# SixLabors/ZlibStream

Hardware: AMD Instinct MI355X
Metric: deflate MB/s (input) at level 6, 64 MiB buffers (higher is better)
Workload: dtype u8; 1 GPU; english64: 1 x 67108864-byte pseudo-random-English (Zipf words of alice29.txt) buffer per GPU, level 6, zlib framing, inputs resident in HBM; level=6, buffer_bytes=67108864, buffers_per_gpu=1, compressed_bytes=27425826, parallelism=independent buffers, 1 GPU(s), no collective in the data path

## Files before the change

zlibstream_amd/csrc/zs_engine.hip:

```cpp
#include <hip/hip_runtime.h>

#include <algorithm>
#include <cstdio>
#include <cstdlib>
#include <cstring>
#include <string>
#include <thread>
#include <vector>

#define ZS_BUILDING_LIBRARY
#include "../../include/zsgpu.h"
#include "zs_kernels.hip"
#include "zs_inflate_par.hip"
#include "zs_inflate_tok.hip"
#include "zs_png.hip"
#include "zs_crc32.hip"

using namespace zs;

namespace {

struct DevBuf {
    void *p = nullptr;
    size_t cap = 0;
};

enum Stage {
    kStClear, kStAdler, kStLinks, kStMatch, kStChunkMap, kStSegMap, kStResolve, kStExpand, kStEmitSyms, kStTail, kStTrees,
    kStOffsets, kStEmitBits, kStSpecWalk, kStSpecVerify, kStCrc32, kStSpecCompact, kStPngExpand, kStPngSplit, kStPngPack, kStPngSurvey, kStPngCompose, kStPngDiff, kStPngCrop, kStCount
};
const char *const kStageNames[kStCount] = {"clear", "adler", "links", "match", "chunkmap", "segmap", "resolve", "expand",
                                           "emit_syms", "tail", "trees", "offsets", "emit_bits", "spec_walk", "spec_verify", "crc32_frame",
                                           "spec_compact", "png_expand", "png_split", "png_pack", "png_survey", "png_compose", "png_diff", "png_crop"};

}

struct zs_ctx {
    int device = 0;
    hipStream_t stream = nullptr;
    hipStream_t aux = nullptr;
    hipEvent_t ev_fork = nullptr, ev_join = nullptr, ev_pre0 = nullptr, ev_pre = nullptr;
    hipEvent_t ev_spec[4] = {};
    std::string err;
    bool profiling = false;
    int fast_fallbacks = 0;
    int round_runs = 0;
    int cut_rounds = 0;
    int lit_fallbacks = 0;
    int spec_streams = 0, spec_fallbacks = 0, spec_wrong_chunks = 0;
    int spec_periodic = 0;
    int64_t dbg_blk_off = 0, dbg_chunk_off = 0, dbg_nchunks = 0, dbg_spec_n = 0, dbg_n_spec = 0;
    int64_t lit_engine_bytes = 0;
    std::vector<int64_t> inf_used;
    int64_t *inf_probe = nullptr;
    int inf_lane_streams = 0;
    int inf_wave_streams = 0;
    int64_t png_segments = 0;
    int fast_rounds = 0;
    bool no_rounds_once = false;
    int last_op = 0;
    hipEvent_t ev[kStCount + 1] = {};
    double stage_ms[kStCount] = {};
    uint32_t *crc_tab = nullptr;
    DevBuf sd, st, work, wpre, geo, link, mm, maps, chunk_far, segmap, supmap, seg_entry, seg_symbase, seg_stale, entry, symbase, stale, syms, blk_end, blk_top, blocks, trees, info, tile_bits, pieces, scratch,
        stage_in, stage_out, wr, inf_desc, inf_state, par_ps, par_st, par_work, par_cbits, par_ccnt, par_surv, par_scnt, par_cands, par_tabs, par_toktabs, par_toks, par_ctoks, par_tokstat, par_tails, par_retry, par_fxtab, par_blocks, par_cells,
        par_windows, par_fail, run_syms, run_bits, run_scratch, run_outs, run_fail, adl_tr, adl_res, plan_blk, ins_bits, mm_bak, cut_pos, cut_bkt, win_groups, win_sg, win_maps, win_entries, persist_bak, resume_flag, rle_tiles, own_in, fr_chunks, fr_meta, fr_planes, fr_prov, fr_base, fr_counters, spec_rec, spec_flags, spec_syms, png_img, png_seg, png_ctr, png_fimg, png_scratch, png_a7img, png_inflated, png_passes, crc_desc, crc_res, png_zs, png_gather, png_ximg, png_raw, png_simg, png_split, png_gimg, png_vimg, png_vrec, png_packed, png_cimg, png_frames, png_dimg, png_drec, png_kimg, png_crop;
    uint32_t *crc32_tab = nullptr;
    hipEvent_t ev_crc[2] = {};
    hipEvent_t ev_expand[2] = {};
    hipEvent_t ev_split[2] = {};
    hipEvent_t ev_pack[2] = {};
    hipEvent_t ev_survey[2] = {};
    hipEvent_t ev_compose[2] = {};
    hipEvent_t ev_diff[2] = {};
    hipEvent_t ev_crop[2] = {};
    bool resume_poisoned = false;
    void *pinned = nullptr;
    size_t pinned_cap = 0;
    void *pin_io = nullptr;
    size_t pin_io_cap = 0;
    bool pin_io_busy = false;
    void *pin_out = nullptr;
    size_t pin_out_cap = 0;
    bool pin_out_busy = false;
};

namespace {

bool fail(zs_ctx *c, const char *what, hipError_t e) {
    c->err = std::string(what) + ": " + hipGetErrorString(e);
    return false;
}
#define ZS_HIP(c, call)                                  \
    do {                                                 \
        hipError_t e_ = (call);                          \
        if (e_ != hipSuccess) return fail(c, #call, e_); \
    } while (0)

bool ensure(zs_ctx *c, DevBuf &b, size_t bytes) {
    if (bytes <= b.cap) return true;
    if (b.p) (void)hipFree(b.p);
    b.p = nullptr;
    b.cap = 0;
    size_t want = bytes + bytes / 8 + 4096;
    if (hipMalloc(&b.p, want) != hipSuccess) {
        (void)hipGetLastError();
        b.p = nullptr;
        want = bytes + 4096;
        if (hipMalloc(&b.p, want) != hipSuccess) {
            (void)hipGetLastError();
            b.p = nullptr;
            char msg[160];
            snprintf(msg, sizeof msg, "workspace: %zu bytes do not fit the device's free memory (the pipeline needs ~17 bytes per input byte: split the batch)", bytes);
            c->err = msg;
            return false;
        }
    }
    b.cap = want;
    return true;
}
bool ensure_pinned(zs_ctx *c, size_t bytes) {
    if (bytes <= c->pinned_cap) return true;
    if (c->pinned) (void)hipHostFree(c->pinned);
    c->pinned = nullptr;
    c->pinned_cap = 0;
    ZS_HIP(c, hipHostMalloc(&c->pinned, bytes + 4096, hipHostMallocDefault));
    c->pinned_cap = bytes + 4096;
    return true;
}

struct WorkList {
    std::vector<int32_t> pre;
    void add(int stream, int64_t count) {
        while ((int)pre.size() <= stream) pre.push_back(pre.empty() ? 0 : pre.back());
        pre.push_back(pre.back() + (int32_t)count);
    }
    void finish(int n) {
        if (pre.empty()) pre.push_back(0);
        while ((int)pre.size() <= n) pre.push_back(pre.back());
    }
    size_t size() const { return pre.empty() ? 0 : (size_t)pre.back(); }
    bool empty() const { return size() == 0; }
};
constexpr int kWorkLists = 9;
struct Plan {
    std::vector<StreamDesc> sd;
    WorkList w_clear, w_adler, w_links, w_match, w_chunks, w_segs, w_sups, w_blocks, w_runs;
    int64_t n_pos = 0, n_syms = 0;
    int64_t n_chunks = 0, n_segs = 0, n_sups = 0, n_blocks = 0, n_pieces = 0, n_runs = 0;
    int64_t n_spec = 0;
    int max_spec_n = 0, n_spec_streams = 0;
    bool any_fv = false, any_rle = false;
    bool any_dual = false;
    int64_t n_rle_tiles = 0;
    int64_t lit_bytes = 0;
    std::vector<FsChunk> fr_chunks;
    size_t fr_prov = 0;
    int fr_max_n = 0;
    int64_t n_cuts = 0;
    std::vector<int32_t> seg_c0, seg_after, seg_base, seg_S, seg_cl, cstart, head;
    std::vector<uint32_t> cl;
    std::vector<BlockRec> plan_blk;
    std::vector<int32_t> plan_wr_blk;
};

template <class T>
T *dev(DevBuf &b) {
    return (T *)b.p;
}

struct WriteSpec {
    std::vector<int64_t> ends;
    std::vector<uint8_t> flush;
    int chunk = 512;
    bool raw = false;
    bool flushing() const {
        for (uint8_t f : flush)
            if (f) return true;
        return false;
    }
};

struct RunOpts {
    bool final_run = true, cont = false;
    int64_t hist = 0;
    LitPersist *persist = nullptr;
    int64_t abs_off = 0;
    uint32_t adler_stream = 1, carry_byte = 0;
    int64_t end_bits = 0;
    int64_t stop_abs = -1;
    bool resume = false, mid_write = false, at_read = false;
    int64_t p0 = 0, E0 = 0, base0 = 0, start_block = 0;
    int slot = 0;
    uint32_t start_syms = 0;
};

bool run_pipeline(zs_ctx *c, int n, const void *const *in, const int64_t *in_len, void *const *out, const int64_t *out_cap,
                  int64_t *out_len, int *status, int level, int strategy, int hash_variant, hipStream_t stream,
                  const WriteSpec *const *writes = nullptr, int force_seq = 0, RunOpts *ro = nullptr, bool rounds = false,
                  const std::vector<uint8_t> *force_lit = nullptr) {
    if (level == -1) level = 6;
    LevelCfg lv = level_cfg(level);
    static const bool host_times = getenv("ZS_HOST_TIMES") != nullptr;
    const auto ht0 = std::chrono::steady_clock::now();
    auto ht_us = [&]() { return std::chrono::duration<double, std::micro>(std::chrono::steady_clock::now() - ht0).count(); };
    double ht_plan = 0, ht_launched = 0;
    for (int i = 0; i < n; i++) {
        out_len[i] = 0;
        if (status) status[i] = ZS_STREAM_ERROR;
    }
    bool any_writes = false;
    for (int i = 0; i < n && writes; i++) any_writes = any_writes || writes[i] != nullptr;
    if (any_writes && n > 1)
        for (int i = 0; i < n; i++)
            if (ro || (writes[i] && writes[i]->flushing())) {
                c->err = "flush modes and incremental runs take one stream a call";
                return false;
            }
    std::vector<WriteSpec> rle_one;
    std::vector<const WriteSpec *> rle_writes;
    if (any_writes && strategy == kRle && level >= 1 && !ro && !getenv("ZS_NO_RLE_MULTI")) {
        rle_one.resize((size_t)n);
        rle_writes.assign(writes, writes + n);
        for (int i = 0; i < n; i++) {
            const WriteSpec *wr = writes[i];
            if (!wr || wr->ends.size() <= 1 || wr->flushing()) continue;
            bool safe = true;
            for (size_t k = 0; k + 1 < wr->ends.size() && safe; k++) {
                const int64_t E = wr->ends[k];
                safe = !(E >= kWindowSize - kMinLookahead && (E % kWSize) >= kWSize - kMinLookahead);
            }
            if (safe) {
                rle_one[(size_t)i] = *wr;
                rle_one[(size_t)i].ends.assign(1, in_len[i]);
                rle_one[(size_t)i].flush.assign(1, 0);
                rle_writes[(size_t)i] = &rle_one[(size_t)i];
            }
        }
        writes = rle_writes.data();
    }
    static const int64_t fast_min_input = getenv("ZS_FAST_MIN_INPUT") ? atoll(getenv("ZS_FAST_MIN_INPUT")) : kFastMinPeriodic;
    bool allow_dual = lv.func == 1 && strategy != kRle && strategy != kHuffmanOnly && !any_writes && !ro && !rounds && force_seq == 0 && !force_lit && n <= 16 && !getenv("ZS_NO_FAST_VEC") &&
                      !getenv("ZS_FAST_NO_ROUNDS");
    for (int i = 0; i < n && allow_dual; i++) allow_dual = in_len[i] >= fast_min_input && in_len[i] < kFastMinInput;
    bool dual_broken = false;
    const bool spec_on = !getenv("ZS_NO_SPEC");
    const int spec_len_env = getenv("ZS_SPEC_LEN") ? atoi(getenv("ZS_SPEC_LEN")) : 0;
    const int spec_bits = spec_len_env == 512 ? 9 : spec_len_env == 2048 ? 11 : spec_len_env == 1024 ? 10 : kSpecLenBits;
    const int spec_warm = getenv("ZS_SPEC_WARM") ? std::max(0, std::min(4096, atoi(getenv("ZS_SPEC_WARM")))) : kSpecWarm;
    const int64_t spec_min = getenv("ZS_SPEC_MIN") ? std::max<int64_t>(kWindowSize, atoll(getenv("ZS_SPEC_MIN"))) : kSpecMinInput;
    const int spec_corrupt = getenv("ZS_SPEC_CORRUPT") ? atoi(getenv("ZS_SPEC_CORRUPT")) : -1;
plan_again:
    Plan pl;
    pl.sd.resize((size_t)n);
    int64_t total_len = 0;
    for (int i = 0; i < n; i++) total_len += in_len[i];
    const int64_t link_span = total_len >= (48ll << 20) ? 262144 : total_len >= (24ll << 20) ? 131072 : 65536;
    const int run_chunk = getenv("ZS_FAST_CHUNK") ? std::max(65536, std::min((int)kFastChunk, atoi(getenv("ZS_FAST_CHUNK")) & ~65535))
                                                  : (int)std::max<int64_t>(65536, std::min<int64_t>(kFastChunk, ((total_len / 256 + 65535) >> 16) << 16));
    for (int i = 0; i < n; i++) {
        StreamDesc &s = pl.sd[(size_t)i];
        int64_t len = in_len[i];
        const WriteSpec *const wr = writes ? writes[i] : nullptr;
        s.in = (const uint8_t *)in[i];
        s.out = (uint8_t *)out[i];
        s.out_cap = out_cap[i];
        s.n = (int32_t)len;
        const bool multi = wr && wr->ends.size() > 1;
        const bool flushing = wr && (wr->flushing() || ro);
        const bool resume = ro && ro->resume;
        const bool cont = ro && ro->cont && !resume, final_run = !ro || ro->final_run;
        std::vector<ReadEvent> rev;
        Geometry geo;
        const int64_t one_write[1] = {len};
        const bool real_flush = wr && wr->flushing();
        const bool lit_forced = force_lit && (*force_lit)[(size_t)i];
        const std::vector<int64_t> no_ends_;
        GeoStart gs;
        if (resume) gs.resume = true, gs.at_read = ro->at_read, gs.p0 = ro->p0, gs.E0 = ro->E0, gs.base0 = ro->base0;
        bool inner_flush = false;
        if (wr)
            for (size_t k = 0; k + 1 < wr->flush.size(); k++) inner_flush = inner_flush || wr->flush[k] != 0;
        const bool slow_ok = lv.func == 2 && strategy != kRle && !cont && !lit_forced && !(multi && inner_flush) &&
                             build_geometry(len, multi ? wr->ends : no_ends_, geo, gs);
        const bool fast_multi = multi && !inner_flush && !cont && !resume && lv.func == 1 && strategy != kRle && !getenv("ZS_NO_FAST_MULTI") &&
                                build_read_events(len, wr->ends, rev, true);
        const bool fast_resume = resume && ro->at_read && lv.func == 1 && strategy != kRle && !inner_flush && !lit_forced && !getenv("ZS_NO_FAST_RESUME") &&
                                 len - ro->p0 >= 2 * kMinLookahead &&
                                 (multi ? build_read_events(len, wr->ends, rev, true, ro->p0, ro->base0)
                                        : build_read_events(len, std::vector<int64_t>(one_write, one_write + 1), rev, true, ro->p0, ro->base0));
        const bool regular = fast_resume ? true : cont ? false : multi ? fast_multi : build_read_events(len, std::vector<int64_t>(one_write, one_write + 1), rev);
        s.body_end = slow_ok ? (int32_t)geo.body_end : -1;
        const bool fast_one = lv.func == 1 && strategy != kRle && regular && len >= kMinLookahead && !cont && !resume &&
                              ((!flushing && final_run && !ro && (!multi || fast_multi)) || (ro && (!multi || fast_multi) && !inner_flush && !lit_forced && !getenv("ZS_NO_FAST_RESUME")));
        const bool fast_par = fast_one && !multi && force_seq != 1 && !ro && strategy != kHuffmanOnly &&
                              (len >= kFastMinInput || allow_dual || (force_seq == 2 && n <= 16 && len >= fast_min_input));
        if (allow_dual && !fast_par) dual_broken = true;
        s.fv_end = ((fast_one && (!fast_par || allow_dual) && !getenv("ZS_NO_FAST_VEC")) || fast_resume) ? (int32_t)(len - kMinLookahead) : -1;
        s.ins_bits = nullptr;
        if (s.fv_end >= 0) {
            pl.any_fv = true;
        }
        s.rle_end = -1, s.rle_tile_off = 0;
        s.fr_first = 0, s.fr_n = 0;
        if (strategy == kRle && level >= 1 && !multi && !flushing && final_run && !ro && regular && !getenv("ZS_NO_RLE_RUNS")) {
            s.rle_end = (int32_t)rle_body_end(len);
            if (s.rle_end >= 0) {
                pl.any_rle = true;
                s.rle_tile_off = (int32_t)pl.n_rle_tiles;
                pl.n_rle_tiles += (s.rle_end + kMaxMatch + 1 + 4095) / 4096;
            }
        }
        s.n_wr = (multi || flushing) ? (int32_t)wr->ends.size() : 1;
        s.wr_end = nullptr;
        s.wr_flush = nullptr, s.wr_blk = nullptr, s.out_chunk = wr ? wr->chunk : 512, s.raw = wr && wr->raw;
        s.kl = num_refills(len - (resume ? ro->base0 : 0));
        s.resume = resume && (slow_ok || fast_resume) ? 1 : 0, s.cont_bits = (cont || resume) ? 1 : 0, s.mid_write = (ro && (ro->mid_write || (resume && !ro->at_read))) ? 1 : 0;
        if (resume && !slow_ok && !fast_resume) {
            c->err = "the run cannot go on in the bulk pipeline from where the literal engine stopped";
            return false;
        }
        s.start_slot = resume ? ro->slot : 0, s.start_syms = resume ? ro->start_syms : 0, s.base0 = resume ? ro->base0 : 0;
        s.start_block = resume ? ro->start_block : 0, s.start_pos = resume ? ro->p0 : 0, s.persist_off = resume ? ro->abs_off : 0, s.stop_abs = (ro && cont) ? ro->stop_abs : -1;
        s.nchunks = s.body_end >= 0 ? geo.nchunks() : 0;
        s.pos_off = pl.n_pos;
        pl.n_pos += (len + 64 + 63) & ~63LL;
        s.sym_off = pl.n_syms;
        pl.n_syms += len + 64 + (ro ? kLitBufsize : 0);
        s.chunk_off = (int32_t)pl.n_chunks;
        pl.n_chunks += s.nchunks;
        s.seg_off = (int32_t)pl.n_segs;
        s.nsegs = 0;
        s.cut_off = (int32_t)pl.n_cuts, s.cut_cap = 0;
        s.grid_chunks = 0;
        if (s.body_end >= 0) {
            s.grid_chunks = 1;
            for (size_t k = 1; k + 1 < geo.cstart.size() && s.grid_chunks; k++)
                if (geo.cstart[k] != (int32_t)((int64_t)k * kChunk - (kMinLookahead - 1))) s.grid_chunks = 0;
            if (geo.cstart.empty() || geo.cstart[0] != 0) s.grid_chunks = 0;
            for (size_t k = 0; k < geo.head.size() && s.grid_chunks; k++)
                if (geo.head[k] != ((k >= 32 && ((k - 32) & 15) == 0) ? (int32_t)((k - 32) >> 4) + 2 : 0)) s.grid_chunks = 0;
            s.cut_cap = (int32_t)(geo.cl.size() + (size_t)geo.nsegs() + 8);
            pl.n_cuts += s.cut_cap;
            s.nsegs = geo.nsegs();
            const int32_t cl0 = (int32_t)pl.cl.size();
            pl.seg_c0.insert(pl.seg_c0.end(), geo.seg_c0.begin(), geo.seg_c0.end());
            pl.seg_after.insert(pl.seg_after.end(), geo.seg_after.begin(), geo.seg_after.end());
            pl.seg_base.insert(pl.seg_base.end(), geo.seg_base.begin(), geo.seg_base.end());
            pl.seg_S.insert(pl.seg_S.end(), geo.seg_S.begin(), geo.seg_S.end());
            for (int32_t v : geo.seg_cl) pl.seg_cl.push_back(v + cl0);
            pl.cl.insert(pl.cl.end(), geo.cl.begin(), geo.cl.end());
            pl.cstart.insert(pl.cstart.end(), geo.cstart.begin(), geo.cstart.end());
            pl.head.insert(pl.head.end(), geo.head.begin(), geo.head.end());
        } else {
            if (fast_resume) {
                pl.seg_c0.push_back(0), pl.seg_after.push_back((int32_t)std::max<int64_t>(ro->p0, kMinLookahead - 1)), pl.seg_base.push_back((int32_t)ro->base0);
                pl.seg_S.push_back(0), pl.seg_cl.push_back((int32_t)pl.cl.size());
                s.nsegs++;
            }
            if (s.fv_end >= 0 || s.rle_end >= 0)
                for (size_t k = 0; k < rev.size(); k++) {
                    const int64_t at = (k || fast_resume) ? rev[k].at - (s.rle_end >= 0 ? kMaxMatch : kMinLookahead - 1) : 0;
                    if (at > (s.rle_end >= 0 ? s.rle_end : s.fv_end)) break;
                    pl.seg_c0.push_back(0), pl.seg_after.push_back((int32_t)rev[k].after), pl.seg_base.push_back((int32_t)rev[k].base);
                    pl.seg_S.push_back(0), pl.seg_cl.push_back((int32_t)pl.cl.size());
                    s.nsegs++;
                }
            pl.seg_cl.push_back((int32_t)pl.cl.size());
            pl.cstart.push_back(0);
        }
        s.seg_c0 = s.seg_after = s.seg_base = s.seg_S = s.seg_cl = nullptr, s.cl = nullptr, s.cstart = nullptr, s.head = nullptr;
        pl.n_segs += s.nsegs;
        s.sup_off = (int32_t)pl.n_sups;
        pl.n_sups += (s.nsegs + kSupSegs - 1) / kSupSegs;
        s.spec = 0, s.spec_n = 0, s.spec_off = (int32_t)pl.n_spec;
        bool spec_geo = s.body_end >= 0 && geo.body_end == len - kMinLookahead;
        if (spec_geo) {
            const int64_t want = 1 + (len > kWindowSize ? (len - kWindowSize - 1) / kWSize + 1 : 0);
            spec_geo = (int64_t)geo.nsegs() == want && geo.seg_cl.size() == (size_t)want + 1 && geo.seg_cl[0] == 0 && geo.seg_cl[1] == 0;
            for (int64_t k = 1; k < want && spec_geo; k++)
                spec_geo = geo.seg_cl[(size_t)k + 1] - geo.seg_cl[(size_t)k] == 1 &&
                           geo.cl[(size_t)geo.seg_cl[(size_t)k]] == ((uint32_t)(kWindowSize + kWSize * (k - 1)) | kClWindowBit);
        }
        if (spec_on && lv.func == 2 && (strategy == kDefault || strategy == kFiltered) && !wr && !ro && !lit_forced && spec_geo && len >= spec_min &&
            n <= 65535) {
            s.spec = 1, s.spec_n = (int32_t)((((int64_t)s.body_end + kMinLookahead - 1) >> spec_bits) + 1);
            pl.n_spec += s.spec_n, pl.n_spec_streams++;
            pl.max_spec_n = std::max(pl.max_spec_n, (int)s.spec_n);
        }
        s.run_chunk = run_chunk;
        s.fast_runs = fast_par ? (force_seq == 2 ? 1 : (int32_t)((len + run_chunk - 1) / run_chunk)) : 0;
        s.run_slots = fast_par ? (force_seq == 2 ? (int32_t)((len + 4096) / kFastChunk + 1) : s.fast_runs) : 0;
        s.run_off = (int32_t)pl.n_runs;
        pl.n_runs += s.run_slots;
        pl.w_runs.add(i, s.fast_runs);
        s.blk_off = (int32_t)pl.n_blocks;
        s.max_blocks = (int32_t)(level == 0 ? len / 8191 + len / 32506 + 4 : len / kBlockSyms + 2);
        if (flushing) s.max_blocks += (int32_t)wr->ends.size() + 1;
        s.plan_blk = nullptr, s.plan_nblk = 0;
        s.final_run = final_run ? 1 : 0, s.cont = cont ? 1 : 0, s.persist = ro ? ro->persist : nullptr;
        s.abs_off = (ro && !resume) ? ro->abs_off : 0, s.adler_stream = ro ? ro->adler_stream : 1, s.carry_byte = ro ? ro->carry_byte : 0;
        if (level == 0 && strategy != kRle && !ro) {
            const size_t first = pl.plan_blk.size();
            const std::vector<int64_t> no_ends;
            const std::vector<uint8_t> no_flush;
            if (flushing) pl.plan_wr_blk.assign(wr->ends.size(), 0);
            plan_stored_blocks(len, (multi || flushing) ? wr->ends : no_ends, flushing ? wr->flush : no_flush,
                               [&](int64_t start, int32_t blen, int can_store, int eof) {
                                   pl.plan_blk.push_back(BlockRec{start, 0, blen, 0, can_store, eof});
                               },
                               [&](int w, int nb) {
                                   if (flushing) pl.plan_wr_blk[(size_t)w] = nb;
                               });
            s.plan_nblk = (int32_t)(pl.plan_blk.size() - first);
            s.plan_blk = (const BlockRec *)(uintptr_t)first;
            s.max_blocks = s.plan_nblk + 1;
        }
        pl.n_blocks += s.max_blocks;
        s.adler_off = (int32_t)pl.n_pieces;
        s.n_adler = ro ? 0 : (int32_t)((len + kAdlerPiece - 1) / kAdlerPiece);
        pl.n_pieces += s.n_adler;
        pl.w_clear.add(i, (s.out_cap + 65535) / 65536);
        pl.w_adler.add(i, s.n_adler);
        if (s.body_end >= 0 || s.fast_runs > 0 || s.fv_end >= 0)
            pl.w_links.add(i, len - 5 > 0 ? (len - 5 + link_span - 1) / link_span : 0);
        if (s.body_end >= 0) {
            pl.w_match.add(i, (int64_t)s.body_end / kMatchTile + 1);
            pl.w_chunks.add(i, s.nchunks);
            pl.w_segs.add(i, s.nsegs);
            if (s.nsegs > kSupSegs) pl.w_sups.add(i, (s.nsegs + kSupSegs - 1) / kSupSegs);
        }
        pl.w_blocks.add(i, s.max_blocks);
        if (s.body_end < 0 && s.fv_end < 0 && s.rle_end < 0 && s.fast_runs == 0 && s.plan_nblk == 0 && !(level == 0 && strategy != kRle && !ro)) {
            const int64_t from = resume ? ro->p0 : ro ? ro->hist : 0;
            pl.lit_bytes += std::max<int64_t>(0, len - from - (kMinLookahead - 1));
        }
    }
    {
        int64_t need = 0;
        for (int i = 0; i < n; i++) need += (pl.sd[(size_t)i].spec_n + 63) / 64;
        if (pl.n_spec && (int64_t)((pl.max_spec_n + 63) / 64) * n > 4 * need + 4096) {
            for (int i = 0; i < n; i++) pl.sd[(size_t)i].spec = 0, pl.sd[(size_t)i].spec_n = 0, pl.sd[(size_t)i].spec_off = 0;
            pl.n_spec = 0, pl.max_spec_n = 0, pl.n_spec_streams = 0;
        }
    }
    if (allow_dual && dual_broken) {
        allow_dual = false, dual_broken = false;
        goto plan_again;
    }
    pl.any_dual = allow_dual;
    c->lit_engine_bytes += pl.lit_bytes;
    auto plan_rerun = [&]() { c->lit_engine_bytes -= pl.lit_bytes; };
    c->fast_rounds = 0;
    const bool no_rounds_this_call = c->no_rounds_once;
    c->no_rounds_once = false;
    if (pl.any_fv && !getenv("ZS_FAST_NO_ROUNDS") && !no_rounds_this_call && !(ro && ro->resume && getenv("ZS_NO_RESUME_ROUNDS"))) {
        int64_t pos_fv = 0, max_fv = 0;
        for (int i = 0; i < n; i++)
            if (pl.sd[(size_t)i].fv_end >= 0) {
                pos_fv += pl.sd[(size_t)i].fv_end + 1 - pl.sd[(size_t)i].start_pos;
                max_fv = std::max<int64_t>(max_fv, pl.sd[(size_t)i].fv_end + 1 - pl.sd[(size_t)i].start_pos);
            }
        const double t_stream = (double)max_fv / (level >= 3 ? 20e6 : level == 2 ? 35e6 : 46e6);
        const double t_rounds = std::min(0.016, (double)max_fv / 60e6) + (double)pos_fv / 3.5e9;
        if (getenv("ZS_FR_RATIO") ? (double)pos_fv <= atof(getenv("ZS_FR_RATIO")) * (double)max_fv : t_rounds < t_stream) {
            int64_t target = getenv("ZS_FR_CHUNK") ? atoll(getenv("ZS_FR_CHUNK")) : pos_fv / 250;
            target = target < 2048 ? 2048 : target > kFsChunkMax ? kFsChunkMax : target;
            bool too_short = false;
            for (;;) {
                pl.fr_chunks.clear();
                pl.fr_max_n = 0;
                too_short = false;
                for (int i = 0; i < n; i++) {
                    StreamDesc &s = pl.sd[(size_t)i];
                    if (s.fv_end < 0) continue;
                    s.fr_first = (int32_t)pl.fr_chunks.size();
                    {
                        const int32_t *after = pl.seg_after.data() + s.seg_off;
                        const bool res = s.resume != 0;
                        const int64_t shortest = fs_build_chunks(i, (int64_t)s.fv_end, s.nsegs - 1, [&](int k) { return (int64_t)after[k - 1] - (kMinLookahead - 1); }, (int)target, pl.fr_chunks,
                                                                 res ? 2 : 1, res ? s.start_pos : 0);
                        if (shortest < kFsMinSpan) too_short = true;
                    }
                    s.fr_n = (int32_t)pl.fr_chunks.size() - s.fr_first;
                    pl.fr_max_n = s.fr_n > pl.fr_max_n ? s.fr_n : pl.fr_max_n;
                }
                if (pl.fr_chunks.size() <= 256 || target >= kFsChunkMax || getenv("ZS_FR_CHUNK")) break;
                target += 128;
            }
            if (too_short) {
                pl.fr_chunks.clear();
                pl.fr_max_n = 0;
                for (int i = 0; i < n; i++) pl.sd[(size_t)i].fr_first = pl.sd[(size_t)i].fr_n = 0;
            }
            for (FsChunk &ck : pl.fr_chunks) {
                ck.prov_off = (uint32_t)pl.fr_prov;
                pl.fr_prov += (size_t)(ck.b_hi - ck.b_lo) + kMaxMatch + 64;
            }
            if (pl.fr_prov > 0xFFFF0000u) {
                pl.fr_chunks.clear();
                pl.fr_max_n = 0, pl.fr_prov = 0;
                for (int i = 0; i < n; i++) pl.sd[(size_t)i].fr_first = pl.sd[(size_t)i].fr_n = 0;
            }
        }
    }
    WorkList *const lists[kWorkLists] = {&pl.w_clear, &pl.w_adler, &pl.w_links, &pl.w_match, &pl.w_chunks, &pl.w_segs, &pl.w_sups, &pl.w_blocks, &pl.w_runs};
    for (WorkList *l : lists) l->finish(n);
    size_t n_work = pl.w_clear.size() + pl.w_adler.size() + pl.w_links.size() + pl.w_match.size() + pl.w_chunks.size() +
                    pl.w_segs.size() + pl.w_sups.size() + pl.w_blocks.size() + pl.w_runs.size();
    if (!ensure(c, c->sd, sizeof(StreamDesc) * (size_t)n) || !ensure(c, c->st, sizeof(StreamState) * (size_t)n) ||
        !ensure(c, c->work, sizeof(uint2) * (n_work + 1)) || !ensure(c, c->link, 2 * (size_t)pl.n_pos + 64) ||
        !ensure(c, c->mm, 8 * (size_t)pl.n_pos + 256) ||
        !ensure(c, c->maps, 4 * (size_t)(pl.n_chunks + 1) * kSlots) || !ensure(c, c->segmap, 8 * (size_t)(pl.n_segs + 1) * kSlots) ||
        !ensure(c, c->supmap, 8 * (size_t)(pl.n_sups + 1) * kSlots) || !ensure(c, c->chunk_far, 2 * (size_t)pl.n_chunks + 64) ||
        !ensure(c, c->seg_entry, 2 * (size_t)(pl.n_segs + 2)) || !ensure(c, c->seg_symbase, 4 * (size_t)(pl.n_segs + 2)) ||
        !ensure(c, c->seg_stale, (size_t)pl.n_segs + 64) || !ensure(c, c->entry, 2 * (size_t)(pl.n_chunks + 2)) ||
        !ensure(c, c->symbase, 4 * (size_t)(pl.n_chunks + 2)) || !ensure(c, c->stale, (size_t)pl.n_chunks + 64) ||
        !ensure(c, c->syms, 4 * (size_t)pl.n_syms + kSymsSlack) || !ensure(c, c->blk_end, 4 * (size_t)pl.n_blocks + 64) ||
        !ensure(c, c->blk_top, 4 * (size_t)pl.n_blocks + 64) || !ensure(c, c->blocks, sizeof(BlockRec) * (size_t)pl.n_blocks) ||
        !ensure(c, c->trees, sizeof(TreeWork) * (size_t)pl.n_blocks) || !ensure(c, c->info, sizeof(BlockInfo) * (size_t)pl.n_blocks) ||
        !ensure(c, c->tile_bits, 4 * (size_t)kEbTiles * (size_t)pl.n_blocks + 64) ||
        !ensure(c, c->pieces, 4 * (size_t)pl.n_pieces + 64) || !ensure(c, c->scratch, (size_t)kScratchBytes * (size_t)n) ||
        !ensure(c, c->cut_pos, 8 * (size_t)pl.n_cuts + 64) || !ensure(c, c->cut_bkt, 8 * (size_t)pl.n_cuts + 64) ||
        (pl.n_spec && (!ensure(c, c->spec_rec, 8 * (size_t)pl.n_spec + 64) || !ensure(c, c->spec_flags, 4 * (size_t)n + 64) ||
                       !ensure(c, c->spec_syms, 4 * (size_t)pl.n_spec * (size_t)spec_slab_stride(spec_bits) + 64))))
        return false;
    const size_t o_segcl = 16 * (size_t)pl.n_segs, o_cstart = o_segcl + 4 * ((size_t)pl.n_segs + (size_t)n),
                 o_head = o_cstart + 4 * ((size_t)pl.n_chunks + (size_t)n), o_cl = o_head + 4 * (size_t)pl.n_chunks;
    const size_t geo_bytes = o_cl + 4 * pl.cl.size();
    if (!ensure(c, c->geo, geo_bytes + 64)) return false;
    for (int i = 0; i < n; i++) {
        StreamDesc &s = pl.sd[(size_t)i];
        const int32_t *g = (const int32_t *)c->geo.p;
        const uint8_t *gb = (const uint8_t *)c->geo.p;
        s.seg_c0 = g + s.seg_off, s.seg_after = g + pl.n_segs + s.seg_off, s.seg_base = g + 2 * pl.n_segs + s.seg_off;
        s.seg_S = g + 3 * pl.n_segs + s.seg_off;
        s.seg_cl = (const int32_t *)(gb + o_segcl) + s.seg_off + i;
        s.cstart = (const int32_t *)(gb + o_cstart) + s.chunk_off + i;
        s.head = (const int32_t *)(gb + o_head) + s.chunk_off;
        s.cl = (const uint32_t *)(gb + o_cl);
    }
    if (pl.any_fv) {
        if (!ensure(c, c->ins_bits, (size_t)pl.n_pos / 8 + kFvBitSlack)) return false;
        for (int i = 0; i < n; i++)
            if (pl.sd[(size_t)i].fv_end >= 0) pl.sd[(size_t)i].ins_bits = dev<uint32_t>(c->ins_bits) + pl.sd[(size_t)i].pos_off / 32;
    }
    if (!pl.plan_blk.empty()) {
        if (!ensure(c, c->plan_blk, sizeof(BlockRec) * pl.plan_blk.size())) return false;
        for (int i = 0; i < n; i++)
            if (pl.sd[(size_t)i].plan_nblk) pl.sd[(size_t)i].plan_blk = dev<BlockRec>(c->plan_blk) + (uintptr_t)pl.sd[(size_t)i].plan_blk;
    }
    if (pl.n_runs &&
        (!ensure(c, c->run_syms, 4 * (size_t)pl.n_runs * kFastRunSyms) || !ensure(c, c->run_bits, 4 * (size_t)pl.n_runs * kFastRunBitWords) ||
         !ensure(c, c->run_scratch, (size_t)pl.n_runs * kFastRunScratch) || !ensure(c, c->run_outs, sizeof(FastRunOut) * (size_t)pl.n_runs) ||
         !ensure(c, c->run_fail, 4 * (size_t)n + 64)))
        return false;
    if (any_writes) {
        std::vector<size_t> nws((size_t)n, 0), offs;
        for (int i = 0; i < n; i++) {
            const WriteSpec *wr = writes[i];
            if (wr && (wr->ends.size() > 1 || wr->flushing() || ro)) nws[(size_t)i] = wr->ends.size();
        }
        const size_t wr_bytes = layout_write_blocks(nws, offs);
        if (!ensure(c, c->wr, wr_bytes + 64)) return false;
        std::vector<uint8_t> hw(rounds ? 0 : wr_bytes + 64, 0);
        for (int i = 0; i < n; i++) {
            const WriteSpec *wr = writes[i];
            const size_t nw = nws[(size_t)i];
            if (!wr || !(wr->ends.size() > 1 || wr->flushing() || ro)) continue;
            uint8_t *blk = (uint8_t *)c->wr.p + offs[(size_t)i];
            pl.sd[(size_t)i].wr_end = (const int64_t *)blk;
            if (wr->flushing() || ro) {
                pl.sd[(size_t)i].wr_blk = (int32_t *)(blk + 8 * nw);
                pl.sd[(size_t)i].wr_flush = blk + 12 * nw;
            }
            if (rounds || !nw) continue;
            memcpy(hw.data() + offs[(size_t)i], wr->ends.data(), sizeof(int64_t) * nw);
            if (wr->flushing() || ro) memcpy(hw.data() + offs[(size_t)i] + 12 * nw, wr->flush.data(), nw);
            if (!pl.plan_wr_blk.empty()) memcpy(hw.data() + offs[(size_t)i] + 8 * nw, pl.plan_wr_blk.data(), 4 * nw);
        }
        if (!rounds && wr_bytes) {
            ZS_HIP(c, hipMemcpyAsync(c->wr.p, hw.data(), hw.size(), hipMemcpyHostToDevice, stream));
            ZS_HIP(c, hipStreamSynchronize(stream));
        }
    }
    if (!rounds && !pl.plan_blk.empty()) {
        ZS_HIP(c, hipMemcpyAsync(c->plan_blk.p, pl.plan_blk.data(), sizeof(BlockRec) * pl.plan_blk.size(), hipMemcpyHostToDevice, stream));
        ZS_HIP(c, hipStreamSynchronize(stream));
    }
    const size_t pre_bytes = 4 * (size_t)kWorkLists * (size_t)(n + 1);
    size_t up_bytes = sizeof(StreamDesc) * (size_t)n + pre_bytes + geo_bytes + 16;
    if (!ensure_pinned(c, std::max(up_bytes, sizeof(StreamState) * (size_t)n)) || !ensure(c, c->wpre, pre_bytes + 64)) return false;
    uint8_t *hp = (uint8_t *)c->pinned;
    memcpy(hp, pl.sd.data(), sizeof(StreamDesc) * (size_t)n);
    int32_t *hpre = (int32_t *)(hp + sizeof(StreamDesc) * (size_t)n);
    size_t o_clear = 0, o_adler, o_links, o_match, o_chunks, o_segs, o_sups, o_blocks, o_runs;
    WorkOffsets wo;
    {
        size_t *const offs[kWorkLists] = {&o_clear, &o_adler, &o_links, &o_match, &o_chunks, &o_segs, &o_sups, &o_blocks, &o_runs};
        size_t at = 0;
        for (int l = 0; l < kWorkLists; l++) {
            *offs[l] = at;
            wo.off[l] = (uint32_t)at;
            memcpy(hpre + (size_t)l * (size_t)(n + 1), lists[l]->pre.data(), 4 * (size_t)(n + 1));
            at += lists[l]->size();
        }
        wo.off[kWorkLists] = (uint32_t)at;
    }
    if (geo_bytes) {
        uint8_t *hg = hp + sizeof(StreamDesc) * (size_t)n + pre_bytes;
        if (pl.n_segs) {
            memcpy(hg, pl.seg_c0.data(), 4 * (size_t)pl.n_segs);
            memcpy(hg + 4 * (size_t)pl.n_segs, pl.seg_after.data(), 4 * (size_t)pl.n_segs);
            memcpy(hg + 8 * (size_t)pl.n_segs, pl.seg_base.data(), 4 * (size_t)pl.n_segs);
            memcpy(hg + 12 * (size_t)pl.n_segs, pl.seg_S.data(), 4 * (size_t)pl.n_segs);
        }
        memcpy(hg + o_segcl, pl.seg_cl.data(), 4 * pl.seg_cl.size());
        memcpy(hg + o_cstart, pl.cstart.data(), 4 * pl.cstart.size());
        if (pl.n_chunks) memcpy(hg + o_head, pl.head.data(), 4 * (size_t)pl.n_chunks);
        if (!pl.cl.empty()) memcpy(hg + o_cl, pl.cl.data(), 4 * pl.cl.size());
        if (!rounds) ZS_HIP(c, hipMemcpyAsync(c->geo.p, hg, geo_bytes, hipMemcpyHostToDevice, stream));
    }
    if (!rounds) ZS_HIP(c, hipMemcpyAsync(c->sd.p, hp, sizeof(StreamDesc) * (size_t)n, hipMemcpyHostToDevice, stream));
    if (n_work && !rounds) {
        ZS_HIP(c, hipMemcpyAsync(c->wpre.p, hpre, pre_bytes, hipMemcpyHostToDevice, stream));
        hipLaunchKernelGGL(zs_worklist_kernel, dim3((unsigned)((n_work + 255) / 256)), dim3(256), 0, stream, dev<int32_t>(c->wpre), n, wo,
                           dev<uint2>(c->work));
    }
    if (!rounds) {
        ZeroRegions z;
        auto reg = [&](int r, DevBuf &b, size_t bytes) {
            z.p[r] = b.p;
            z.n16[r] = (uint32_t)(((bytes + 15) / 16 < b.cap / 16) ? (bytes + 15) / 16 : b.cap / 16);
        };
        reg(0, c->stale, (size_t)pl.n_chunks + 64);
        reg(1, c->seg_stale, (size_t)pl.n_segs + 64);
        reg(2, c->st, sizeof(StreamState) * (size_t)n);
        if (pl.any_fv) reg(3, c->ins_bits, (size_t)pl.n_pos / 8 + kFvBitSlack);
        else z.p[3] = nullptr, z.n16[3] = 0;
        uint32_t most = 0;
        for (int r = 0; r < 4; r++) most = z.n16[r] > most ? z.n16[r] : most;
        unsigned blocks = (most + 255) / 256;
        if (blocks > 2048) blocks = 2048;
        if (blocks < 1) blocks = 1;
        hipLaunchKernelGGL(zs_zero_kernel, dim3(blocks), dim3(256), 0, stream, z);
        if (ro && ro->resume && pl.sd[0].fv_end >= 0) {
            const int64_t lo = std::max<int64_t>(0, ro->p0 - kWSize - 64) / 32, hi = ro->p0 / 32;
            if (hi > lo) ZS_HIP(c, hipMemsetAsync(pl.sd[0].ins_bits + lo, 0xFF, (size_t)(hi - lo) * 4, stream));
            ZS_HIP(c, hipMemsetD32Async((hipDeviceptr_t)(pl.sd[0].ins_bits + hi), (int)((1u << (ro->p0 & 31)) - 1u), 1, stream));
        }
    }

    const StreamDesc *d_sd = dev<StreamDesc>(c->sd);
    StreamState *d_st = dev<StreamState>(c->st);
    const uint2 *d_work = dev<uint2>(c->work);
    const bool prof = c->profiling;
    const int k5_ahead = getenv("ZS_K5_AHEAD") ? atoi(getenv("ZS_K5_AHEAD")) : 1;
    c->dbg_blk_off = pl.sd[0].blk_off, c->dbg_chunk_off = pl.sd[0].chunk_off, c->dbg_nchunks = pl.sd[0].nchunks;
    c->dbg_spec_n = pl.sd[0].spec_n, c->dbg_n_spec = pl.n_spec;
    const K5Spec k5s{dev<uint32_t>(c->spec_rec), dev<uint32_t>(c->spec_rec) + pl.n_spec, spec_bits, spec_warm, spec_corrupt,
                     dev<uint32_t>(c->spec_syms), spec_slab_stride(spec_bits)};
    int spec_ok_streams = 0;
    bool need_maps = true, spec_ran = false;
    if (!rounds) c->spec_streams = c->spec_fallbacks = c->spec_wrong_chunks = c->spec_periodic = 0;
    auto mark = [&](int i) {
        if (prof) (void)hipEventRecord(c->ev[i], stream);
    };
    ht_plan = ht_us();
    ZS_HIP(c, hipEventRecord(c->ev_pre0, stream));
    auto side_work = [&]() -> bool {
        ZS_HIP(c, hipStreamWaitEvent(c->aux, c->ev_pre0, 0));
        if (!pl.w_clear.empty())
            hipLaunchKernelGGL(zs_clear_kernel, dim3((unsigned)pl.w_clear.size()), dim3(256), 0, c->aux, d_sd, d_work + o_clear);
        if (!pl.w_adler.empty())
            hipLaunchKernelGGL(zs_adler_kernel, dim3((unsigned)pl.w_adler.size()), dim3(256), 0, c->aux, d_sd, d_work + o_adler,
                               dev<uint32_t>(c->pieces));
        ZS_HIP(c, hipEventRecord(c->ev_pre, c->aux));
        return true;
    };
    const int cut_budget = getenv("ZS_FORCE_ROUNDS") ? 0 : kCutBudget;
    const int defer_mode = ((ro || getenv("ZS_NO_DEFER")) ? 0 : 1) | (getenv("ZS_DEBUG_CUTS") ? 0x100 : 0) | (cut_budget << 16);
    const int cut_stride = (int)pl.n_cuts;
    const bool use_sup = !pl.w_sups.empty() && !getenv("ZS_NO_SUPMAP");
    auto launch_resolve = [&](int mode, int iter) {
        hipLaunchKernelGGL(zs_resolve_kernel, dim3((unsigned)n), dim3(1024), kResolveLds, stream, d_sd, d_st, dev<uint16_t>(c->link),
                           dev<uint2>(c->mm), dev<uint32_t>(c->maps), dev<uint2>(c->segmap),
                           dev<uint16_t>(c->seg_entry), dev<uint32_t>(c->seg_symbase), dev<uint8_t>(c->stale),
                           dev<uint8_t>(c->seg_stale), c->crc_tab, lv, strategy, hash_variant, 0x7FFFFFFF, 0x7FFFFFFF,
                           use_sup ? dev<uint2>(c->supmap) : (const uint2 *)nullptr, dev<uint16_t>(c->chunk_far), mode, dev<int32_t>(c->cut_pos),
                           dev<uint32_t>(c->cut_bkt), cut_stride, iter);
    };
    auto run_cut_rounds = [&]() -> bool {
        const size_t far_off = 8 * (size_t)pl.n_pos + 256;
        if (!ensure(c, c->mm_bak, far_off + 2 * (size_t)pl.n_chunks + 64)) return false;
        ZS_HIP(c, hipMemcpyAsync(c->mm_bak.p, c->mm.p, 8 * (size_t)pl.n_pos + 256, hipMemcpyDeviceToDevice, stream));
        ZS_HIP(c, hipMemcpyAsync((uint8_t *)c->mm_bak.p + far_off, c->chunk_far.p, 2 * (size_t)pl.n_chunks + 64, hipMemcpyDeviceToDevice, stream));
        ZS_HIP(c, hipMemsetAsync(c->cut_pos.p, 0xFF, 8 * (size_t)pl.n_cuts + 64, stream));
        StreamState *hr = (StreamState *)c->pinned;
        for (int iter = 0;; iter++) {
            launch_resolve(3 | (defer_mode & 0x100), iter);
            ZS_HIP(c, hipMemcpyAsync(hr, d_st, sizeof(StreamState) * (size_t)n, hipMemcpyDeviceToHost, stream));
            ZS_HIP(c, hipStreamSynchronize(stream));
            bool all_same = true;
            int max_nc = 0;
            for (int i = 0; i < n; i++)
                if (hr[i].deferred == 1 && !hr[i].cuts_same) all_same = false, max_nc = std::max(max_nc, hr[i].nc[iter & 1]);
            hipLaunchKernelGGL(zs_cuts_apply_kernel, dim3((unsigned)n), dim3(256), 0, stream, d_sd, d_st, dev<uint16_t>(c->link), dev<int32_t>(c->cut_pos),
                               cut_stride, iter);
            if (getenv("ZS_DEBUG")) {
                int nd = 0, nsame = 0;
                for (int i = 0; i < n; i++) nd += hr[i].deferred == 1, nsame += hr[i].deferred == 1 && hr[i].cuts_same;
                fprintf(stderr, "zs: cut round %d: %d streams in the rounds, %d settled, most cuts %d, stream 0: %d cuts, first difference at cut %d (position %d)\n", iter,
                        nd, nsame, max_nc, hr[0].nc[iter & 1], hr[0].cut_diff_idx, hr[0].cut_diff_pos);
            }
            if (all_same && getenv("ZS_DEBUG_CUTS")) {
                const int ncap = hr[0].nc[iter & 1];
                std::vector<int32_t> cp((size_t)ncap);
                std::vector<uint32_t> cb((size_t)ncap);
                (void)hipMemcpy(cp.data(), dev<int32_t>(c->cut_pos) + (size_t)(iter & 1) * (size_t)cut_stride + pl.sd[0].cut_off, 4 * (size_t)ncap, hipMemcpyDeviceToHost);
                (void)hipMemcpy(cb.data(), dev<uint32_t>(c->cut_bkt) + (size_t)(iter & 1) * (size_t)cut_stride + pl.sd[0].cut_off, 4 * (size_t)ncap, hipMemcpyDeviceToHost);
                fprintf(stderr, "zs: cuts of stream 0 (slot: position / bucket):");
                for (int k = 0; k < ncap; k++)
                    if (cp[(size_t)k] >= 0) fprintf(stderr, " %d: %d / %u", k, cp[(size_t)k], cb[(size_t)k]);
                fprintf(stderr, "\n");
            }
            if (all_same) break;
            if (iter >= 4096) {
                c->err = "the cut rounds did not settle";
                return false;
            }
            c->cut_rounds++;
            if (iter > 0)
            hipLaunchKernelGGL(zs_cut_restore_kernel, dim3(2048, (unsigned)std::min(n, 65535)), dim3(256), 0, stream, d_sd, d_st, dev<uint2>(c->mm), (const uint2 *)c->mm_bak.p,
                               dev<uint8_t>(c->stale), dev<uint8_t>(c->seg_stale), dev<uint16_t>(c->chunk_far), (const uint16_t *)((const uint8_t *)c->mm_bak.p + far_off), n);
            if (max_nc > 0) {
                if (max_nc <= 64)
                    hipLaunchKernelGGL((zs_cuts_repair_kernel<256, 1>), dim3(128, (unsigned)max_nc, (unsigned)std::min(n, 65535)), dim3(256), kRepairLds, stream, d_sd, d_st,
                                       dev<uint16_t>(c->link), dev<uint2>(c->mm), dev<uint8_t>(c->stale), dev<uint8_t>(c->seg_stale),
                                       dev<uint16_t>(c->chunk_far), c->crc_tab, lv, hash_variant, dev<int32_t>(c->cut_pos), dev<uint32_t>(c->cut_bkt),
                                       cut_stride, iter, n);
                else if (max_nc <= 2048)
                    hipLaunchKernelGGL((zs_cuts_repair_kernel<256, 8>), dim3(16, (unsigned)max_nc, (unsigned)std::min(n, 65535)), dim3(256), kRepairLds, stream, d_sd, d_st,
                                       dev<uint16_t>(c->link), dev<uint2>(c->mm), dev<uint8_t>(c->stale), dev<uint8_t>(c->seg_stale),
                                       dev<uint16_t>(c->chunk_far), c->crc_tab, lv, hash_variant, dev<int32_t>(c->cut_pos), dev<uint32_t>(c->cut_bkt),
                                       cut_stride, iter, n);
                else
                    hipLaunchKernelGGL((zs_cuts_repair_kernel<1024, 32>), dim3(1, (unsigned)std::min(max_nc, 65535), (unsigned)std::min(n, 65535)), dim3(1024), kRepairLds, stream, d_sd,
                                       d_st, dev<uint16_t>(c->link), dev<uint2>(c->mm), dev<uint8_t>(c->stale), dev<uint8_t>(c->seg_stale),
                                       dev<uint16_t>(c->chunk_far), c->crc_tab, lv, hash_variant, dev<int32_t>(c->cut_pos), dev<uint32_t>(c->cut_bkt),
                                       cut_stride, iter, n);
            }
            hipLaunchKernelGGL(zs_chunkmap_kernel, dim3((unsigned)pl.w_chunks.size()), dim3(512), 0, stream, d_sd, d_work + o_chunks,
                               dev<uint2>(c->mm), dev<uint16_t>(c->link), dev<uint32_t>(c->maps), c->crc_tab, lv, strategy,
                               hash_variant, dev<uint16_t>(c->chunk_far), dev<uint8_t>(c->stale), (const StreamState *)d_st);
            hipLaunchKernelGGL(zs_segmap_kernel, dim3((unsigned)pl.w_segs.size()), dim3(320), 0, stream, d_sd, d_work + o_segs,
                               dev<uint32_t>(c->maps), dev<uint2>(c->segmap));
            ZS_HIP(c, hipMemsetAsync(c->seg_stale.p, 0, (size_t)pl.n_segs + 64, stream));
            if (use_sup)
                hipLaunchKernelGGL(zs_supmap_kernel, dim3((unsigned)pl.w_sups.size()), dim3(320), 0, stream, d_sd, d_work + o_sups,
                                   dev<uint2>(c->segmap), dev<uint8_t>(c->seg_stale), dev<uint2>(c->supmap));
        }
        return true;
    };
    if (!rounds) {
    mark(2);
    if (!pl.w_links.empty())
        hipLaunchKernelGGL(zs_links_kernel, dim3((unsigned)pl.w_links.size()), dim3(1024), kLkLds, stream, d_sd, d_work + o_links,
                           dev<uint16_t>(c->link), c->crc_tab, hash_variant, (int)link_span);
    if (ro && ro->resume)
        hipLaunchKernelGGL(zs_import_chains_kernel, dim3(64), dim3(1024), 0, stream, d_sd, 0, dev<uint16_t>(c->link), c->crc_tab, hash_variant, ro->p0);
    if (pl.any_dual) {
        bool periodic = true;
        if (!getenv("ZS_FAST_NO_PROBE")) {
            hipLaunchKernelGGL(zs_fast_probe_kernel, dim3((unsigned)n), dim3(256), 0, stream, d_sd, dev<uint16_t>(c->link), dev<int32_t>(c->run_fail));
            std::vector<int32_t> np((size_t)n, 0);
            ZS_HIP(c, hipMemcpyAsync(np.data(), c->run_fail.p, 4 * (size_t)n, hipMemcpyDeviceToHost, stream));
            ZS_HIP(c, hipStreamSynchronize(stream));
            for (int i = 0; i < n; i++) periodic = periodic && np[(size_t)i] == 0;
        }
        for (int i = 0; i < n; i++) {
            StreamDesc &sk = pl.sd[(size_t)i];
            if (periodic) sk.fv_end = -1, sk.fr_first = 0, sk.fr_n = 0;
            else sk.fast_runs = 0, sk.run_slots = 0;
        }
        if (periodic) pl.any_fv = false, pl.fr_chunks.clear(), pl.fr_max_n = 0;
        else pl.n_runs = 0;
        memcpy(c->pinned, pl.sd.data(), sizeof(StreamDesc) * (size_t)n);
        ZS_HIP(c, hipMemcpyAsync(c->sd.p, c->pinned, sizeof(StreamDesc) * (size_t)n, hipMemcpyHostToDevice, stream));
        if (getenv("ZS_DEBUG")) fprintf(stderr, "zs: %d stream(s) below 4 MiB at level %d: %s\n", n, level, periodic ? "all period, the speculative runs" : "the sweeps");
    }
    mark(3);
    if (strategy == kHuffmanOnly) {
        ZS_HIP(c, hipMemsetAsync(c->mm.p, 0, 8 * (size_t)pl.n_pos + 64, stream));
    } else if (!pl.w_match.empty())
        hipLaunchKernelGGL(zs_match_kernel, dim3((unsigned)pl.w_match.size()), dim3(1024), kMatchLds + 16, stream, d_sd, d_work + o_match,
                           dev<uint16_t>(c->link), dev<uint2>(c->mm), lv, strategy, d_st);
    mark(4);
    if (!side_work()) return false;
    if (pl.n_spec) {
        spec_ran = true;
        hipLaunchKernelGGL((zs_emit_syms_lane_kernel<4, 1>), dim3((unsigned)((pl.max_spec_n + 63) / 64), (unsigned)n), dim3(kK5Threads), 0, stream, d_sd, d_st,
                           (const uint2 *)nullptr, 0, dev<uint2>(c->mm), dev<uint16_t>(c->link), (const uint16_t *)nullptr, (const uint32_t *)nullptr,
                           (uint32_t *)nullptr, (int32_t *)nullptr, (int32_t *)nullptr, c->crc_tab, lv, strategy, hash_variant, k5_ahead, k5s);
        if (prof) (void)hipEventRecord(c->ev_spec[0], stream);
        hipLaunchKernelGGL(zs_spec_verify_kernel, dim3((unsigned)n), dim3(1024), 0, stream, d_sd, d_st, dev<uint2>(c->mm), dev<uint16_t>(c->link), c->crc_tab, lv,
                           strategy, hash_variant, k5s, dev<int32_t>(c->spec_flags));
        int32_t *hf = (int32_t *)c->pinned;
        ZS_HIP(c, hipMemcpyAsync(hf, c->spec_flags.p, 4 * (size_t)n, hipMemcpyDeviceToHost, stream));
        ZS_HIP(c, hipStreamSynchronize(stream));
        if (prof) (void)hipEventRecord(c->ev_spec[1], stream);
        for (int i = 0; i < n; i++) {
            if (hf[i] == 0) continue;
            c->spec_streams++;
            if (hf[i] == 1) spec_ok_streams++;
            else c->spec_fallbacks++;
            if (hf[i] == 2) c->spec_periodic++;
        }
        if (spec_ok_streams < c->spec_streams) {
            StreamState *hs = (StreamState *)c->pinned;
            ZS_HIP(c, hipMemcpyAsync(hs, d_st, sizeof(StreamState) * (size_t)n, hipMemcpyDeviceToHost, stream));
            ZS_HIP(c, hipStreamSynchronize(stream));
            for (int i = 0; i < n; i++) c->spec_wrong_chunks += hs[i].spec_wrong;
        }
        if (getenv("ZS_DEBUG"))
            fprintf(stderr, "zs: speculative walk: %d streams tried, %d verified, %d wrong guesses (chunks of %d, warm-up %d)\n", c->spec_streams, spec_ok_streams,
                    c->spec_wrong_chunks, 1 << spec_bits, spec_warm);
    }
    need_maps = spec_ok_streams < n;
    const StreamState *spec_st = spec_ok_streams ? (const StreamState *)d_st : nullptr;
    if (!pl.w_chunks.empty() && need_maps)
        hipLaunchKernelGGL(zs_chunkmap_kernel, dim3((unsigned)pl.w_chunks.size()), dim3(512), 0, stream, d_sd, d_work + o_chunks,
                           dev<uint2>(c->mm), dev<uint16_t>(c->link), dev<uint32_t>(c->maps), c->crc_tab, lv, strategy,
                           hash_variant, dev<uint16_t>(c->chunk_far), (uint8_t *)nullptr, (const StreamState *)nullptr, spec_st);
    mark(5);
    if (!pl.w_segs.empty() && need_maps)
        hipLaunchKernelGGL(zs_segmap_kernel, dim3((unsigned)pl.w_segs.size()), dim3(320), 0, stream, d_sd, d_work + o_segs,
                           dev<uint32_t>(c->maps), dev<uint2>(c->segmap), spec_st);
    if (use_sup && need_maps)
        hipLaunchKernelGGL(zs_supmap_kernel, dim3((unsigned)pl.w_sups.size()), dim3(320), 0, stream, d_sd, d_work + o_sups,
                           dev<uint2>(c->segmap), dev<uint8_t>(c->seg_stale), dev<uint2>(c->supmap), spec_st);
    mark(6);
    if (need_maps) launch_resolve(defer_mode, 0);
    }
    mark(7);
    if (pl.any_fv) {
        constexpr int fs_lds = fs_lds_bytes<1024, kFsTile1>();
        if (!pl.fr_chunks.empty()) {
            const size_t nch = pl.fr_chunks.size(), plane_words = (size_t)pl.n_pos / 32 + kFvBitSlack / 4 + 64;
            static const int env_max_rounds = getenv("ZS_FR_MAX_ROUNDS") ? atoi(getenv("ZS_FR_MAX_ROUNDS")) : 0;
            static const int env_range = getenv("ZS_FR_RANGE") ? std::max(1, atoi(getenv("ZS_FR_RANGE"))) : 0;
            static const int env_group = getenv("ZS_FR_GROUP") ? atoi(getenv("ZS_FR_GROUP")) : 4;
            static const int env_tail = getenv("ZS_FR_TAIL_RANGE") ? atoi(getenv("ZS_FR_TAIL_RANGE")) : 1;
            static const bool env_no_seed = getenv("ZS_FR_NO_SEED") != nullptr, env_fixed = getenv("ZS_FR_RANGE_FIXED") != nullptr, env_dbg = getenv("ZS_DEBUG") != nullptr;
            const int max_rounds = env_max_rounds ? env_max_rounds : pl.fr_max_n + 2;
            if (!ensure(c, c->fr_chunks, nch * sizeof(FsChunk)) || !ensure(c, c->fr_meta, 2 * nch * sizeof(FsMeta)) || !ensure(c, c->fr_planes, 16 * plane_words) ||
                !ensure(c, c->fr_prov, 4 * pl.fr_prov + 64) || !ensure(c, c->fr_base, 4 * nch + 64) || !ensure(c, c->fr_counters, 4 * ((size_t)max_rounds + 16))) {
                c->err.clear();
                ZS_HIP(c, hipStreamSynchronize(c->aux));
                ZS_HIP(c, hipStreamSynchronize(stream));
                c->no_rounds_once = true;
                return plan_rerun(), run_pipeline(c, n, in, in_len, out, out_cap, out_len, status, level, strategy, hash_variant, stream, writes, force_seq, ro, false, force_lit);
            }
            ZS_HIP(c, hipMemcpyAsync(c->fr_chunks.p, pl.fr_chunks.data(), nch * sizeof(FsChunk), hipMemcpyHostToDevice, stream));
            ZS_HIP(c, hipMemsetAsync(c->fr_counters.p, 0, 4 * ((size_t)max_rounds + 16), stream));
            const int range_max = env_range ? env_range : nch >= 512 ? (int)((nch + 255) / 256) : 1;
            FsRounds fr{dev<FsChunk>(c->fr_chunks), dev<FsMeta>(c->fr_meta), dev<uint32_t>(c->fr_planes), dev<uint32_t>(c->fr_prov), dev<uint32_t>(c->fr_counters),
                        (int64_t)plane_words, (int)nch, 0, env_no_seed ? 1 : 0, range_max};
            const int group = env_group;
            uint32_t changed = 1;
            int r = 0;
            std::string trace;
            while (r < max_rounds && changed) {
                const int g_n = fr.range > 1 ? 1 : group;
                const unsigned n_wg = (unsigned)((nch + (size_t)fr.range - 1) / (size_t)fr.range);
                for (int g = 0; g < g_n && r < max_rounds; g++, r++) {
                    fr.round = r;
                    hipLaunchKernelGGL((zs_fast_sweep_kernel<1024, kFsTile1, true>), dim3(n_wg), dim3(1024), fs_lds, stream, d_sd, d_st, dev<uint16_t>(c->link),
                                       dev<uint32_t>(c->syms), dev<int32_t>(c->blk_end), dev<int32_t>(c->blk_top), lv, strategy, fr);
                }
                ZS_HIP(c, hipMemcpyAsync(&changed, dev<uint32_t>(c->fr_counters) + (r - 1), 4, hipMemcpyDeviceToHost, stream));
                ZS_HIP(c, hipStreamSynchronize(stream));
                if (env_dbg) {
                    static auto t_last = std::chrono::steady_clock::now();
                    const auto t_now = std::chrono::steady_clock::now();
                    char b[64];
                    snprintf(b, sizeof b, " %u/%d(%.2f)", changed, fr.range, r <= g_n ? 0.0 : std::chrono::duration<double, std::milli>(t_now - t_last).count());
                    t_last = t_now;
                    trace += b;
                }
                if (!env_fixed) {
                    static const double env_wake = getenv("ZS_FR_WAKE") ? atof(getenv("ZS_FR_WAKE")) : 4.0;
                    const size_t awake = std::min<size_t>(nch, (size_t)(env_wake * (double)changed));
                    const int tail = env_tail;
                    fr.range = std::min<int>(range_max, std::max<int>(tail, (int)((awake + 255) / 256)));
                }
            }
            c->fast_rounds = r;
            if (env_dbg) fprintf(stderr, "zs: DeflateFast over %zu chunks of %d streams, up to %d to a workgroup: %d rounds (changed/range:%s)\n", nch, n, range_max, r, trace.c_str());
            if (changed) {
                ZS_HIP(c, hipStreamSynchronize(c->aux));
                c->no_rounds_once = true;
                return plan_rerun(), run_pipeline(c, n, in, in_len, out, out_cap, out_len, status, level, strategy, hash_variant, stream, writes, force_seq, ro, false, force_lit);
            }
            const FsMeta *mf = dev<FsMeta>(c->fr_meta) + (size_t)((r - 1) & 1) * nch;
            hipLaunchKernelGGL(zs_fast_commit_scan_kernel, dim3((unsigned)n), dim3(1024), 0, stream, d_sd, d_st, mf, dev<int32_t>(c->fr_base));
            hipLaunchKernelGGL(zs_fast_commit_kernel, dim3((unsigned)nch), dim3(256), 0, stream, d_sd, fr, mf, dev<int32_t>(c->fr_base), dev<uint16_t>(c->link),
                               dev<uint32_t>(c->syms), dev<int32_t>(c->blk_end), dev<int32_t>(c->blk_top));
        } else {
            hipLaunchKernelGGL((zs_fast_sweep_kernel<1024, kFsTile1, false>), dim3((unsigned)n), dim3(1024), fs_lds, stream, d_sd, d_st, dev<uint16_t>(c->link),
                               dev<uint32_t>(c->syms), dev<int32_t>(c->blk_end), dev<int32_t>(c->blk_top), lv, strategy, FsRounds());
        }
    }
    if (pl.any_rle) {
        const size_t nt = (size_t)pl.n_rle_tiles;
        if (!ensure(c, c->rle_tiles, 4 * (4 * nt + (size_t)n) + 256)) return false;
        int32_t *rb = dev<int32_t>(c->rle_tiles);
        RleTiles rt{rb, rb + nt, rb + 2 * nt, rb + 3 * nt, rb + 4 * nt};
        int max_tiles = 0;
        for (int i = 0; i < n; i++)
            if (pl.sd[(size_t)i].rle_end >= 0) max_tiles = std::max(max_tiles, (pl.sd[(size_t)i].rle_end + kMaxMatch + 1 + 4095) / 4096);
        auto tiles = [&](auto &&launch) {
            for (int s0 = 0; s0 < n; s0 += 65535) launch(dim3((unsigned)((max_tiles + 3) / 4), (unsigned)std::min(n - s0, 65535)), s0);
        };
        tiles([&](dim3 tg, int s0) { hipLaunchKernelGGL(zs_rle_starts_kernel, tg, dim3(256), 0, stream, d_sd, rt, s0); });
        hipLaunchKernelGGL(zs_rle_scan_kernel, dim3((unsigned)n), dim3(1024), 0, stream, d_sd, rt);
        tiles([&](dim3 tg, int s0) {
            hipLaunchKernelGGL(zs_rle_pass_kernel<0>, tg, dim3(256), 0, stream, d_sd, rt, dev<uint32_t>(c->syms), dev<int32_t>(c->blk_end), dev<int32_t>(c->blk_top), s0);
        });
        hipLaunchKernelGGL(zs_rle_sums_kernel, dim3((unsigned)n), dim3(1024), 0, stream, d_sd, d_st, rt);
        tiles([&](dim3 tg, int s0) {
            hipLaunchKernelGGL(zs_rle_pass_kernel<1>, tg, dim3(256), 0, stream, d_sd, rt, dev<uint32_t>(c->syms), dev<int32_t>(c->blk_end), dev<int32_t>(c->blk_top), s0);
        });
    }
    const bool tail_late = ro && (!ro->final_run || ro->resume);
    const bool tail_serial = !tail_late && n >= 64 && (pl.n_pos / n >= (96 << 10) || getenv("ZS_TAIL_SERIAL")) && !getenv("ZS_TAIL_FORK");
    if (!tail_late && !tail_serial) {
        ZS_HIP(c, hipEventRecord(c->ev_fork, stream));
        ZS_HIP(c, hipStreamWaitEvent(c->aux, c->ev_fork, 0));
        hipLaunchKernelGGL(zs_tail_kernel, dim3((unsigned)n), dim3(1024), kTailLds, c->aux, d_sd, d_st, dev<uint16_t>(c->link),
                           dev<uint32_t>(c->syms), dev<int32_t>(c->blk_end), dev<int32_t>(c->blk_top), dev<BlockRec>(c->blocks),
                           dev<uint8_t>(c->scratch), c->crc_tab, lv, strategy, hash_variant, level);
        ZS_HIP(c, hipEventRecord(c->ev_join, c->aux));
    }
    if (!pl.w_segs.empty() && need_maps)
        hipLaunchKernelGGL(zs_expand_kernel, dim3((unsigned)((pl.w_segs.size() + 63) / 64)), dim3(64), 0, stream, d_sd, d_st,
                           d_work + o_segs, (int)pl.w_segs.size(), dev<uint2>(c->mm), dev<uint16_t>(c->link),
                           dev<uint32_t>(c->maps), dev<uint16_t>(c->seg_entry), dev<uint32_t>(c->seg_symbase),
                           dev<uint8_t>(c->stale), dev<uint16_t>(c->entry), dev<uint32_t>(c->symbase), c->crc_tab, lv, strategy,
                           hash_variant);
    mark(8);
    if (!pl.w_chunks.empty() && need_maps)
        hipLaunchKernelGGL((zs_emit_syms_lane_kernel<4, 0>), dim3((unsigned)((pl.w_chunks.size() + 63) / 64)), dim3(kK5Threads), 0, stream, d_sd, d_st,
                           d_work + o_chunks, (int)pl.w_chunks.size(), dev<uint2>(c->mm), dev<uint16_t>(c->link), dev<uint16_t>(c->entry),
                           dev<uint32_t>(c->symbase), dev<uint32_t>(c->syms), dev<int32_t>(c->blk_end), dev<int32_t>(c->blk_top),
                           c->crc_tab, lv, strategy, hash_variant, k5_ahead, k5s);
    if (spec_ok_streams) {
        if (prof) (void)hipEventRecord(c->ev_spec[2], stream);
        hipLaunchKernelGGL(zs_spec_compact_kernel, dim3((unsigned)((pl.max_spec_n + 3) / 4), (unsigned)n), dim3(256), 0, stream, d_sd, d_st, k5s,
                           dev<uint32_t>(c->syms), dev<int32_t>(c->blk_end), dev<int32_t>(c->blk_top));
        if (prof) (void)hipEventRecord(c->ev_spec[3], stream);
    }
    mark(9);
    if (tail_serial)
        hipLaunchKernelGGL(zs_tail_kernel, dim3((unsigned)n), dim3(1024), kTailLds, stream, d_sd, d_st, dev<uint16_t>(c->link),
                           dev<uint32_t>(c->syms), dev<int32_t>(c->blk_end), dev<int32_t>(c->blk_top), dev<BlockRec>(c->blocks),
                           dev<uint8_t>(c->scratch), c->crc_tab, lv, strategy, hash_variant, level);
    else if (!tail_late) ZS_HIP(c, hipStreamWaitEvent(stream, c->ev_join, 0));
    hipLaunchKernelGGL(zs_body_blocks_kernel, dim3((unsigned)n), dim3(256), 0, stream, d_sd, d_st, dev<int32_t>(c->blk_end),
                       dev<int32_t>(c->blk_top), dev<BlockRec>(c->blocks), dev<uint32_t>(c->syms));
    if (tail_late)
        hipLaunchKernelGGL(zs_tail_kernel, dim3((unsigned)n), dim3(1024), kTailLds, stream, d_sd, d_st, dev<uint16_t>(c->link),
                           dev<uint32_t>(c->syms), dev<int32_t>(c->blk_end), dev<int32_t>(c->blk_top), dev<BlockRec>(c->blocks),
                           dev<uint8_t>(c->scratch), c->crc_tab, lv, strategy, hash_variant, level);
    if (pl.n_runs) {
        if (!getenv("ZS_FAST_NO_PROBE") && force_seq == 0 && !pl.any_dual) {
            hipLaunchKernelGGL(zs_fast_probe_kernel, dim3((unsigned)n), dim3(256), 0, stream, d_sd, dev<uint16_t>(c->link), dev<int32_t>(c->run_fail));
            std::vector<int32_t> np((size_t)n, 0);
            ZS_HIP(c, hipMemcpyAsync(np.data(), c->run_fail.p, 4 * (size_t)n, hipMemcpyDeviceToHost, stream));
            ZS_HIP(c, hipStreamSynchronize(stream));
            for (int i = 0; i < n; i++)
                if (np[(size_t)i]) {
                    ZS_HIP(c, hipStreamSynchronize(c->aux));
                    return plan_rerun(), run_pipeline(c, n, in, in_len, out, out_cap, out_len, status, level, strategy, hash_variant, stream, writes, 1, ro, false, force_lit);
                }
        }
        ZS_HIP(c, hipMemsetAsync(c->run_fail.p, 0, 4 * (size_t)n + 64, stream));
        hipLaunchKernelGGL(zs_fast_run_kernel, dim3((unsigned)pl.w_runs.size()), dim3(1024), kFastRunLds, stream, d_sd, d_work + o_runs,
                           dev<uint16_t>(c->link), dev<uint32_t>(c->run_syms), dev<uint32_t>(c->run_bits), dev<uint8_t>(c->run_scratch),
                           dev<FastRunOut>(c->run_outs), c->crc_tab, lv, strategy, hash_variant);
        hipLaunchKernelGGL(zs_fast_verify_kernel, dim3((unsigned)pl.w_runs.size()), dim3(256), 0, stream, d_sd, d_work + o_runs,
                           dev<uint32_t>(c->run_bits), dev<FastRunOut>(c->run_outs), dev<int32_t>(c->run_fail));
        std::vector<int32_t> rfail((size_t)n, 0);
        ZS_HIP(c, hipMemcpyAsync(rfail.data(), c->run_fail.p, 4 * (size_t)n, hipMemcpyDeviceToHost, stream));
        ZS_HIP(c, hipStreamSynchronize(stream));
        for (int i = 0; i < n; i++)
            if (rfail[(size_t)i]) {
                ZS_HIP(c, hipStreamSynchronize(c->aux));
                c->fast_fallbacks++;
                std::vector<FastRunOut> outs((size_t)pl.n_runs);
                ZS_HIP(c, hipMemcpy(outs.data(), c->run_outs.p, sizeof(FastRunOut) * outs.size(), hipMemcpyDeviceToHost));
                if (getenv("ZS_DEBUG"))
                    for (int j = 0; j < pl.sd[(size_t)i].fast_runs; j++) {
                        const FastRunOut &o = outs[(size_t)pl.sd[(size_t)i].run_off + j];
                        fprintf(stderr, "zs: stream %d run %d ok=%d mark=%lld (+%lld syms) end=%lld nsyms=%lld n_ev=%d\n", i, j, o.ok,
                                (long long)o.mark_pos, (long long)o.mark_nsyms, (long long)o.end_pos, (long long)o.nsyms, o.n_ev);
                    }
                double t_engine = 0, t_sweeps = 0;
                for (int k = 0; k < n; k++) {
                    const StreamDesc &sk = pl.sd[(size_t)k];
                    if (sk.fast_runs <= 0) continue;
                    int64_t syms = 0, matches = 0;
                    for (int j = 0; j < sk.fast_runs; j++) syms += outs[(size_t)sk.run_off + j].nsyms, matches += outs[(size_t)sk.run_off + j].n_match;
                    const double scale = sk.fast_runs > 1 ? 0.8 : 1.0;
                    const double te = scale * (1.2e-6 * (double)matches + 0.03e-6 * (double)(syms - matches)) + (double)sk.n / 1.5e9;
                    if (getenv("ZS_DEBUG")) fprintf(stderr, "zs: stream %d: ~%.0f symbols one at a time, ~%.0f in runs of literals, %d bytes\n", k, scale * (double)matches, scale * (double)(syms - matches), sk.n);
                    t_engine = std::max(t_engine, te);
                    t_sweeps = std::max(t_sweeps, (double)sk.n / (level >= 3 ? 20e6 : level == 2 ? 35e6 : 46e6));
                }
                const int mode = (force_seq == 0 && !getenv("ZS_NO_WHOLE_RUNS") && (getenv("ZS_WHOLE_RUNS") || t_engine < 0.7 * t_sweeps)) ? 2 : 1;
                if (getenv("ZS_DEBUG")) fprintf(stderr, "zs: the runs did not verify: %s (engine %.1f ms, sweeps up to %.1f ms)\n", mode == 2 ? "one run per stream" : "the sweeps", t_engine * 1e3, t_sweeps * 1e3);
                return plan_rerun(), run_pipeline(c, n, in, in_len, out, out_cap, out_len, status, level, strategy, hash_variant, stream, writes, mode, ro, false, force_lit);
            }
        hipLaunchKernelGGL(zs_fast_plan_kernel, dim3((unsigned)n), dim3(256), 0, stream, d_sd, d_st, dev<FastRunOut>(c->run_outs), n);
        hipLaunchKernelGGL(zs_fast_stitch_kernel, dim3((unsigned)pl.w_runs.size()), dim3(256), 0, stream, d_sd, d_work + o_runs,
                           dev<uint32_t>(c->run_syms), dev<FastRunOut>(c->run_outs), dev<uint32_t>(c->syms), dev<int32_t>(c->blk_end),
                           dev<int32_t>(c->blk_top));
        hipLaunchKernelGGL(zs_fast_blocks_kernel, dim3((unsigned)n), dim3(64), 0, stream, d_sd, d_st, dev<FastRunOut>(c->run_outs),
                           dev<int32_t>(c->blk_end), dev<int32_t>(c->blk_top), dev<BlockRec>(c->blocks), n);
    }
    mark(10);
    const int trees_threads = pl.w_blocks.size() > 8192 ? 128 : 256;
    if (n >= 64 && !getenv("ZS_NO_LIVE_LIST")) {
        hipLaunchKernelGGL(zs_live_scan_kernel, dim3(1), dim3(1024), 0, stream, d_st, n, dev<int32_t>(c->wpre));
        hipLaunchKernelGGL(zs_live_fill_kernel, dim3((unsigned)((pl.w_blocks.size() + 255) / 256)), dim3(256), 0, stream, dev<int32_t>(c->wpre), n,
                           (uint32_t)pl.w_blocks.size(), dev<uint2>(c->work) + o_blocks);
    }
    hipLaunchKernelGGL(zs_trees_kernel, dim3((unsigned)pl.w_blocks.size()), dim3(trees_threads), 0, stream, d_sd, d_st, d_work + o_blocks,
                       dev<uint32_t>(c->syms), dev<BlockRec>(c->blocks), dev<TreeWork>(c->trees), dev<BlockInfo>(c->info), dev<int32_t>(c->tile_bits), strategy, level);
    mark(11);
    ZS_HIP(c, hipStreamWaitEvent(stream, c->ev_pre, 0));
    hipLaunchKernelGGL(zs_offsets_kernel, dim3((unsigned)n), dim3(256), 0, stream, d_sd, d_st, dev<BlockRec>(c->blocks),
                       dev<BlockInfo>(c->info), dev<TreeWork>(c->trees), dev<uint32_t>(c->pieces), level, n);
    mark(12);
    int eb_tiles = kEbTiles;
    if (level != 0) {
        int64_t longest = 0;
        for (int i = 0; i < n; i++) longest = std::max(longest, in_len[i]);
        eb_tiles = (int)std::min<int64_t>(kEbTiles, (longest + 1) / kEbTile + 1);
    }
    static const char *const eb_env = getenv("ZS_EB_TILES");
    if (eb_env) eb_tiles = std::max(1, std::min(kEbTiles, atoi(eb_env)));
    hipLaunchKernelGGL(zs_emit_bits_kernel, dim3((unsigned)pl.w_blocks.size(), (unsigned)(1 + eb_tiles)), dim3(256), 0, stream, d_sd, d_st,
                       d_work + o_blocks, dev<uint32_t>(c->syms), dev<BlockRec>(c->blocks), dev<TreeWork>(c->trees), dev<BlockInfo>(c->info),
                       dev<int32_t>(c->tile_bits));
    mark(13);
    ZS_HIP(c, hipGetLastError());
    StreamState *hst = (StreamState *)c->pinned;
    ZS_HIP(c, hipMemcpyAsync(hst, d_st, sizeof(StreamState) * (size_t)n, hipMemcpyDeviceToHost, stream));
    ht_launched = ht_us();
    ZS_HIP(c, hipStreamSynchronize(stream));
    if (host_times) fprintf(stderr, "zs: host: plan + uploads %.0f us, all launched at %.0f us, device done at %.0f us\n", ht_plan, ht_launched, ht_us());
    c->last_op = lv.func == 1 ? 2 : 0;
    if (getenv("ZS_DEBUG_CHAIN") && n == 1) {
        const int64_t q0 = atoll(getenv("ZS_DEBUG_CHAIN")) - (ro ? ro->abs_off : 0);
        if (q0 > 0 && q0 < in_len[0]) {
            std::vector<uint16_t> lk((size_t)in_len[0]);
            (void)hipMemcpy(lk.data(), dev<uint16_t>(c->link) + pl.sd[0].pos_off, 2 * (size_t)in_len[0], hipMemcpyDeviceToHost);
            fprintf(stderr, "[zs] run of %lld bytes (stream position %lld on), resume %d at %lld: chain of %lld:", (long long)in_len[0], (long long)(ro ? ro->abs_off : 0),
                    pl.sd[0].resume, (long long)pl.sd[0].start_pos, (long long)q0);
            int64_t q = q0;
            int hops = 0;
            const int64_t want = getenv("ZS_DEBUG_CHAIN_WANT") ? atoll(getenv("ZS_DEBUG_CHAIN_WANT")) - (ro ? ro->abs_off : 0) : -1;
            int want_at = -1;
            while (lk[(size_t)q] && hops < 100000) {
                q -= lk[(size_t)q], hops++;
                if (hops <= 12) fprintf(stderr, " %lld", (long long)q);
                if (q == want) want_at = hops;
            }
            fprintf(stderr, " ... %d hops, ends at %lld; position %lld is hop %d\n", hops, (long long)q, (long long)want, want_at);
        }
    }
    if (getenv("ZS_DEBUG_FA") && writes && writes[0] && pl.sd[0].wr_blk) {
        const WriteSpec *wr = writes[0];
        const size_t nw = wr->ends.size();
        std::vector<int32_t> wb(nw);
        (void)hipMemcpy(wb.data(), pl.sd[0].wr_blk, 4 * nw, hipMemcpyDeviceToHost);
        fprintf(stderr, "[zs] run of %lld bytes, %zu Writes, %d blocks, body ends at %d, resume %d; blocks before each Write:", (long long)in_len[0], nw, hst[0].nblocks,
                pl.sd[0].body_end, pl.sd[0].resume);
        for (size_t k = 0; k < nw && k < 24; k++) fprintf(stderr, " %d(end %lld, flush %d)", wb[k], (long long)wr->ends[k], wr->flush.empty() ? 0 : wr->flush[k]);
        fprintf(stderr, "\n");
    }
    if (prof) {
        for (int i = 0; i < kStCount; i++) {
            float ms = 0;
            if (i >= kStLinks && i <= kStEmitBits) (void)hipEventElapsedTime(&ms, c->ev[i], c->ev[i + 1]);
            c->stage_ms[i] = ms;
        }
        if (spec_ran) {
            float a = 0, b = 0, m = 0;
            (void)hipEventElapsedTime(&a, c->ev[kStChunkMap], c->ev_spec[0]);
            (void)hipEventElapsedTime(&b, c->ev_spec[0], c->ev_spec[1]);
            (void)hipEventElapsedTime(&m, c->ev_spec[1], c->ev[kStChunkMap + 1]);
            c->stage_ms[kStSpecWalk] = a, c->stage_ms[kStSpecVerify] = b, c->stage_ms[kStChunkMap] = m;
            float k = 0;
            if (spec_ok_streams) (void)hipEventElapsedTime(&k, c->ev_spec[2], c->ev_spec[3]);
            c->stage_ms[kStSpecCompact] = k;
        }
    }
    {
        bool any_poison = false;
        std::vector<uint8_t> fl(force_lit ? *force_lit : std::vector<uint8_t>((size_t)n, 0));
        for (int i = 0; i < n; i++)
            if (hst[i].poison) any_poison = true, fl[(size_t)i] = 1;
        if (any_poison) {
            ZS_HIP(c, hipStreamSynchronize(c->aux));
            if (ro && ro->resume) {
                c->err = "the resumed run met a read the bulk pipeline leaves to the literal engine";
                c->resume_poisoned = true;
                return false;
            }
            c->lit_fallbacks++;
            return plan_rerun(), run_pipeline(c, n, in, in_len, out, out_cap, out_len, status, level, strategy, hash_variant, stream, writes, force_seq, ro, false, &fl);
        }
    }
    if (!ro && !rounds) {
        bool gave_up = false;
        for (int i = 0; i < n; i++) gave_up = gave_up || hst[i].deferred == 1;
        if (gave_up) {
            ZS_HIP(c, hipStreamSynchronize(c->aux));
            c->round_runs++;
            if (!run_cut_rounds()) return false;
            return plan_rerun(), run_pipeline(c, n, in, in_len, out, out_cap, out_len, status, level, strategy, hash_variant, stream, writes, force_seq, ro, true, force_lit);
        }
    }
    if (ro) ro->end_bits = hst[0].end_bits;
    bool all_ok = true;
    for (int i = 0; i < n; i++) {
        out_len[i] = hst[i].out_len;
        if (status) status[i] = hst[i].status;
        if (hst[i].status != 0 && all_ok) {
            c->err = hst[i].status == ZS_BUF_ERROR ? "buffer error"
                                                   : "stored block larger than the reference's pending buffer (the managed engine throws here)";
            all_ok = false;
        }
    }
    return all_ok;
}

bool device_adlers(zs_ctx *c, int m, const void *const *bufs, const int64_t *lens, const void *const *trailers, uint32_t *adlers,
                   int *ok, hipStream_t stream) {
    if (m <= 0) return true;
    std::vector<StreamDesc> sd((size_t)m);
    std::vector<uint2> work;
    int64_t n_pieces = 0;
    for (int i = 0; i < m; i++) {
        StreamDesc &s = sd[(size_t)i];
        memset(&s, 0, sizeof s);
        s.in = (const uint8_t *)bufs[i];
        s.n = (int32_t)lens[i];
        s.adler_off = (int32_t)n_pieces;
        s.n_adler = (int32_t)((lens[i] + kAdlerPiece - 1) / kAdlerPiece);
        n_pieces += s.n_adler;
        for (int k = 0; k < s.n_adler; k++) work.push_back(make_uint2((unsigned)i, (unsigned)k));
    }
    const size_t b_sd = sizeof(StreamDesc) * (size_t)m, b_work = sizeof(uint2) * work.size(), b_tr = sizeof(void *) * (size_t)m;
    if (!ensure(c, c->sd, b_sd) || !ensure(c, c->work, b_work + 16) || !ensure(c, c->pieces, 4 * (size_t)n_pieces + 64) ||
        !ensure(c, c->adl_tr, b_tr) || !ensure(c, c->adl_res, sizeof(uint2) * (size_t)m) ||
        !ensure_pinned(c, b_sd + b_work + b_tr + sizeof(uint2) * (size_t)m))
        return false;
    uint8_t *hp = (uint8_t *)c->pinned;
    memcpy(hp, sd.data(), b_sd);
    if (b_work) memcpy(hp + b_sd, work.data(), b_work);
    if (trailers) memcpy(hp + b_sd + b_work, trailers, b_tr);
    ZS_HIP(c, hipMemcpyAsync(c->sd.p, hp, b_sd, hipMemcpyHostToDevice, stream));
    if (b_work) ZS_HIP(c, hipMemcpyAsync(c->work.p, hp + b_sd, b_work, hipMemcpyHostToDevice, stream));
    if (trailers) ZS_HIP(c, hipMemcpyAsync(c->adl_tr.p, hp + b_sd + b_work, b_tr, hipMemcpyHostToDevice, stream));
    if (!work.empty())
        hipLaunchKernelGGL(zs_adler_kernel, dim3((unsigned)work.size()), dim3(256), 0, stream, dev<StreamDesc>(c->sd), dev<uint2>(c->work),
                           dev<uint32_t>(c->pieces));
    hipLaunchKernelGGL(zs_adler_finish_kernel, dim3((unsigned)m), dim3(256), 0, stream, dev<StreamDesc>(c->sd), dev<uint32_t>(c->pieces),
                       trailers ? (const uint8_t *const *)c->adl_tr.p : nullptr, dev<uint2>(c->adl_res));
    uint2 *hres = (uint2 *)(hp + b_sd + b_work + b_tr);
    ZS_HIP(c, hipMemcpyAsync(hres, c->adl_res.p, sizeof(uint2) * (size_t)m, hipMemcpyDeviceToHost, stream));
    ZS_HIP(c, hipStreamSynchronize(stream));
    for (int i = 0; i < m; i++) {
        if (adlers) adlers[i] = hres[i].x;
        if (ok) ok[i] = (int)hres[i].y;
    }
    return true;
}

int batch_prefix_that_fits(zs_ctx *c, int n, const int64_t *in_len, const int64_t *out_cap, int lo, int per_byte) {
    size_t free_b = 0, total_b = 0;
    if (hipMemGetInfo(&free_b, &total_b) != hipSuccess) return n;
    const DevBuf *held[] = {&c->link, &c->mm, &c->maps, &c->segmap, &c->supmap, &c->syms, &c->trees, &c->blocks, &c->info, &c->tile_bits, &c->stage_in, &c->stage_out,
                            &c->scratch, &c->ins_bits, &c->mm_bak};
    size_t have = 0;
    for (const DevBuf *b : held) have += b->cap;
    const double budget = 0.55 * ((double)free_b + (double)have);
    double need = 0;
    int hi = lo;
    while (hi < n) {
        const double add = (double)in_len[hi] * per_byte + (per_byte > 19 ? (double)out_cap[hi] : 0.0) + 4.0e6;
        if (hi > lo && need + add > budget) break;
        need += add;
        hi++;
    }
    return hi;
}

bool check_args(zs_ctx *c, int n, const int64_t *in_len, int level, int strategy) {
    if (!c) return false;
    if (n < 0 || level < -1 || level > 9 || strategy < 0 || strategy > 4) {
        c->err = "stream error";
        return false;
    }
    for (int i = 0; i < n; i++)
        if (in_len[i] < 0 || in_len[i] > 0x7FFFFFFF - 1024) {
            c->err = "stream error";
            return false;
        }
    return true;
}

}

extern "C" {

void zs_ctx_destroy(zs_ctx *c);
int zs_ctx_create(int device, zs_ctx **out) {
    if (!out) return ZS_STREAM_ERROR;
    *out = nullptr;
    int count = 0;
    if (hipGetDeviceCount(&count) != hipSuccess || count <= 0 || device < 0 || device >= count) return ZS_STREAM_ERROR;
    if (hipSetDevice(device) != hipSuccess) return ZS_STREAM_ERROR;
    zs_ctx *c = new zs_ctx();
    c->device = device;
    if (hipStreamCreateWithFlags(&c->stream, hipStreamNonBlocking) != hipSuccess) {
        zs_ctx_destroy(c);
        return ZS_MEM_ERROR;
    }
    for (auto &e : c->ev) (void)hipEventCreate(&e);
    for (auto &e : c->ev_spec) (void)hipEventCreate(&e);
    for (auto &e : c->ev_crc) (void)hipEventCreate(&e);
    for (auto &e : c->ev_expand) (void)hipEventCreate(&e);
    for (auto &e : c->ev_compose) (void)hipEventCreate(&e);
    for (auto &e : c->ev_diff) (void)hipEventCreate(&e);
    for (auto &e : c->ev_crop) (void)hipEventCreate(&e);
    for (auto &e : c->ev_split) (void)hipEventCreate(&e);
    for (auto &e : c->ev_pack) (void)hipEventCreate(&e);
    for (auto &e : c->ev_survey) (void)hipEventCreate(&e);
    {
        int *d_ok = nullptr, ok = 0;
        if (hipMalloc((void **)&d_ok, sizeof(int)) != hipSuccess) {
            zs_ctx_destroy(c);
            return ZS_MEM_ERROR;
        }
        hipLaunchKernelGGL(zs_lds_order_kernel, dim3(1), dim3(64), 0, c->stream, d_ok);
        const bool copied = hipMemcpyAsync(&ok, d_ok, sizeof(int), hipMemcpyDeviceToHost, c->stream) == hipSuccess &&
                            hipStreamSynchronize(c->stream) == hipSuccess;
        (void)hipFree(d_ok);
        if (!copied || !ok) {
            fprintf(stderr, "zsgpu: LDS lane-order self-test failed on device %d; this build cannot run there\n", device);
            zs_ctx_destroy(c);
            return ZS_STREAM_ERROR;
        }
    }
    if (hipStreamCreateWithFlags(&c->aux, hipStreamNonBlocking) != hipSuccess ||
        hipEventCreateWithFlags(&c->ev_fork, hipEventDisableTiming) != hipSuccess ||
        hipEventCreateWithFlags(&c->ev_join, hipEventDisableTiming) != hipSuccess ||
        hipEventCreateWithFlags(&c->ev_pre0, hipEventDisableTiming) != hipSuccess ||
        hipEventCreateWithFlags(&c->ev_pre, hipEventDisableTiming) != hipSuccess) {
        zs_ctx_destroy(c);
        return ZS_MEM_ERROR;
    }
    std::vector<uint32_t> tab(1024);
    for (int t = 0; t < 4; t++)
        for (int i = 0; i < 256; i++) tab[(size_t)t * 256 + i] = crc32c_table_entry(t, (uint32_t)i);
    if (hipMalloc((void **)&c->crc_tab, 4096) != hipSuccess ||
        hipMemcpy(c->crc_tab, tab.data(), 4096, hipMemcpyHostToDevice) != hipSuccess ||
        hipFuncSetAttribute((const void *)zs_match_kernel, hipFuncAttributeMaxDynamicSharedMemorySize, kMatchLds + 16) != hipSuccess ||
        hipFuncSetAttribute((const void *)zs_resolve_kernel, hipFuncAttributeMaxDynamicSharedMemorySize, kResolveLds) != hipSuccess ||
        hipFuncSetAttribute((const void *)zs_links_kernel, hipFuncAttributeMaxDynamicSharedMemorySize, kLkLds) != hipSuccess ||
        hipFuncSetAttribute((const void *)zs_tail_kernel, hipFuncAttributeMaxDynamicSharedMemorySize, kTailLds) != hipSuccess ||
        hipFuncSetAttribute((const void *)zs_fast_run_kernel, hipFuncAttributeMaxDynamicSharedMemorySize, kFastRunLds) != hipSuccess ||
        hipFuncSetAttribute((const void *)zs_fast_sweep_kernel<1024, kFsTile1, false>, hipFuncAttributeMaxDynamicSharedMemorySize, (fs_lds_bytes<1024, kFsTile1>())) != hipSuccess ||
        hipFuncSetAttribute((const void *)zs_fast_sweep_kernel<1024, kFsTile1, true>, hipFuncAttributeMaxDynamicSharedMemorySize, (fs_lds_bytes<1024, kFsTile1>())) != hipSuccess ||
        hipFuncSetAttribute((const void *)zs_inf_window_kernel, hipFuncAttributeMaxDynamicSharedMemorySize, kWinMapLds) != hipSuccess ||
        hipFuncSetAttribute((const void *)zs_inf_chain_par_kernel, hipFuncAttributeMaxDynamicSharedMemorySize, kChainParLds) != hipSuccess ||
        hipFuncSetAttribute((const void *)zs_inf_expand_kernel, hipFuncAttributeMaxDynamicSharedMemorySize, kExpLds) != hipSuccess ||
        hipFuncSetAttribute((const void *)zs_cuts_repair_kernel<256, 1>, hipFuncAttributeMaxDynamicSharedMemorySize, kRepairLds) != hipSuccess ||
        hipFuncSetAttribute((const void *)zs_cuts_repair_kernel<256, 8>, hipFuncAttributeMaxDynamicSharedMemorySize, kRepairLds) != hipSuccess ||
        hipFuncSetAttribute((const void *)zs_cuts_repair_kernel<1024, 32>, hipFuncAttributeMaxDynamicSharedMemorySize, kRepairLds) != hipSuccess ||
        hipFuncSetAttribute((const void *)zs_png_unfilter_kernel, hipFuncAttributeMaxDynamicSharedMemorySize, kPngMaxLds) != hipSuccess ||
        hipFuncSetAttribute((const void *)zs_inflate_kernel, hipFuncAttributeMaxDynamicSharedMemorySize, kInfLds) != hipSuccess) {
        zs_ctx_destroy(c);
        return ZS_MEM_ERROR;
    }
    hipFuncAttributes fa;
    if (hipFuncGetAttributes(&fa, (const void *)zs_match_kernel) != hipSuccess || fa.sharedSizeBytes != 0) {
        fprintf(stderr, "zsgpu: zs_match_kernel has static LDS; its tile addressing assumes none\n");
        zs_ctx_destroy(c);
        return ZS_STREAM_ERROR;
    }
    *out = c;
    return ZS_OK;
}

void zs_ctx_destroy(zs_ctx *c) {
    if (!c) return;
    (void)hipSetDevice(c->device);
    DevBuf *bufs[] = {&c->sd, &c->st, &c->work, &c->wpre, &c->geo, &c->link, &c->mm, &c->maps, &c->chunk_far, &c->segmap, &c->supmap, &c->seg_entry, &c->seg_symbase, &c->seg_stale, &c->entry, &c->symbase, &c->stale, &c->syms,
                      &c->blk_end, &c->blk_top, &c->blocks, &c->trees, &c->info, &c->tile_bits, &c->pieces, &c->scratch, &c->stage_in, &c->stage_out, &c->wr, &c->inf_desc, &c->inf_state, &c->par_ps, &c->par_st, &c->par_work, &c->par_cbits, &c->par_ccnt, &c->par_surv, &c->par_scnt,
                      &c->par_cands, &c->par_tabs, &c->par_toktabs, &c->par_toks, &c->par_ctoks, &c->par_tokstat, &c->par_tails, &c->par_retry, &c->par_fxtab, &c->par_blocks, &c->par_cells, &c->par_windows, &c->par_fail, &c->run_syms, &c->run_bits,
                      &c->run_scratch, &c->run_outs, &c->run_fail, &c->adl_tr, &c->adl_res, &c->plan_blk, &c->ins_bits, &c->mm_bak, &c->cut_pos, &c->cut_bkt, &c->win_groups, &c->win_sg, &c->win_maps, &c->win_entries, &c->persist_bak, &c->resume_flag, &c->rle_tiles, &c->own_in, &c->fr_chunks, &c->fr_meta, &c->fr_planes, &c->fr_prov, &c->fr_base, &c->fr_counters, &c->spec_rec, &c->spec_flags, &c->spec_syms, &c->png_img, &c->png_seg, &c->png_ctr, &c->png_fimg, &c->png_scratch, &c->png_a7img, &c->png_inflated, &c->png_passes, &c->crc_desc, &c->crc_res, &c->png_zs, &c->png_gather, &c->png_ximg, &c->png_raw, &c->png_simg, &c->png_split, &c->png_gimg, &c->png_vimg, &c->png_vrec, &c->png_packed, &c->png_cimg, &c->png_frames, &c->png_dimg, &c->png_drec, &c->png_kimg, &c->png_crop};
    for (DevBuf *b : bufs)
        if (b->p) (void)hipFree(b->p);
    if (c->crc_tab) (void)hipFree(c->crc_tab);
    if (c->crc32_tab) (void)hipFree(c->crc32_tab);
    for (auto &e : c->ev_crc)
        if (e) (void)hipEventDestroy(e);
    for (auto &e : c->ev_expand)
        if (e) (void)hipEventDestroy(e);
    for (auto &e : c->ev_split)
        if (e) (void)hipEventDestroy(e);
    for (auto &e : c->ev_pack)
        if (e) (void)hipEventDestroy(e);
    for (auto &e : c->ev_survey)
        if (e) (void)hipEventDestroy(e);
    for (auto &e : c->ev_compose)
        if (e) (void)hipEventDestroy(e);
    for (auto &e : c->ev_diff)
        if (e) (void)hipEventDestroy(e);
    for (auto &e : c->ev_crop)
        if (e) (void)hipEventDestroy(e);
    if (c->pinned) (void)hipHostFree(c->pinned);
    if (c->pin_io) (void)hipHostFree(c->pin_io);
    if (c->pin_out) (void)hipHostFree(c->pin_out);
    for (auto &e : c->ev)
        if (e) (void)hipEventDestroy(e);
    for (auto &e : c->ev_spec)
        if (e) (void)hipEventDestroy(e);
    if (c->ev_fork) (void)hipEventDestroy(c->ev_fork);
    if (c->ev_join) (void)hipEventDestroy(c->ev_join);
    if (c->ev_pre0) (void)hipEventDestroy(c->ev_pre0);
    if (c->ev_pre) (void)hipEventDestroy(c->ev_pre);
    if (c->aux) (void)hipStreamDestroy(c->aux);
    if (c->stream) (void)hipStreamDestroy(c->stream);
    delete c;
}

const char *zs_ctx_last_error(const zs_ctx *c) { return c ? c->err.c_str() : "no context"; }

int64_t zs_deflate_bound(int64_t n) { return n + (n >> 3) + 1024; }

void zs_ctx_set_profiling(zs_ctx *c, int enable) {
    if (c) c->profiling = enable != 0;
}
int zs_ctx_stage_count(const zs_ctx *) { return kStCount; }
int64_t zs_ctx_counter(const zs_ctx *c, const char *name) {
    if (!c || !name) return -1;
    const std::string k(name);
    if (k == "fast_rounds") return c->fast_rounds;
    if (k == "fast_fallbacks") return c->fast_fallbacks;
    if (k == "round_runs") return c->round_runs;
    if (k == "cut_rounds") return c->cut_rounds;
    if (k == "lit_fallbacks") return c->lit_fallbacks;
    if (k == "lit_engine_bytes") return c->lit_engine_bytes;
    if (k == "spec_streams") return c->spec_streams;
    if (k == "spec_fallbacks") return c->spec_fallbacks;
    if (k == "spec_periodic") return c->spec_periodic;
    if (k == "spec_wrong_chunks") return c->spec_wrong_chunks;
    if (k == "inf_lane_streams") return c->inf_lane_streams;
    if (k == "inf_wave_streams") return c->inf_wave_streams;
    if (k == "png_segments") return c->png_segments;
    return -1;
}

int64_t zs_ctx_debug_read(zs_ctx *c, const char *name, void *out, int64_t cap) {
    if (!c || !name || !out || !c->st.p) return -1;
    const std::string k(name);
    (void)hipSetDevice(c->device);
    StreamState ss;
    if (hipMemcpy(&ss, c->st.p, sizeof ss, hipMemcpyDeviceToHost) != hipSuccess) return -1;
    const void *src = nullptr;
    int64_t bytes = 0;
    const int32_t state[6] = {ss.tail_p, ss.tail_kind, (int32_t)ss.tail_pend, ss.k_done, ss.preins, (int32_t)ss.body_syms};
    if (k == "state") {
        if (cap < (int64_t)sizeof state) return -1;
        memcpy(out, state, sizeof state);
        return sizeof state;
    }
    if (k == "blk_end") src = dev<int32_t>(c->blk_end) + c->dbg_blk_off, bytes = 4 * (int64_t)(ss.body_syms / kBlockSyms);
    else if (k == "blk_top") src = dev<int32_t>(c->blk_top) + c->dbg_blk_off, bytes = 4 * (int64_t)(ss.body_syms / kBlockSyms);
    else if (k == "symbase") src = dev<uint32_t>(c->symbase) + c->dbg_chunk_off, bytes = 4 * c->dbg_nchunks;
    else if (k == "spec_base") src = dev<uint32_t>(c->spec_rec) + c->dbg_n_spec, bytes = 4 * c->dbg_spec_n;
    else return -1;
    if (bytes > cap || (bytes > 0 && !src)) return -1;
    if (bytes > 0 && hipMemcpy(out, src, (size_t)bytes, hipMemcpyDeviceToHost) != hipSuccess) return -1;
    return bytes;
}

const char *zs_ctx_stage_name(const zs_ctx *c, int s) {
    static const char *const inf_names[6] = {"inf_find", "inf_measure", "inf_chain", "inf_decode", "inf_windows", "inf_resolve"};
    if (s == kStCrc32 || s == kStSpecCompact || s == kStPngExpand || s == kStPngSplit || s == kStPngPack || s == kStPngSurvey || s == kStPngCompose || s == kStPngDiff || s == kStPngCrop) return kStageNames[s];
    if (c && c->last_op == 1) return s >= 0 && s < 6 ? inf_names[s] : "";
    if (c && c->last_op == 2 && s == kStExpand) return "fast_sweep";
    if (c && c->last_op == 2 && s == kStTail) return "fast_runs+tail";
    return s >= 0 && s < kStCount ? kStageNames[s] : "";
}
double zs_ctx_stage_ms(const zs_ctx *c, int s) { return c && s >= 0 && s < kStCount ? c->stage_ms[s] : 0.0; }

int zs_deflate_batch_device(zs_ctx *c, int n, const void *const *in, const int64_t *in_len, void *const *out,
                            const int64_t *out_cap, int64_t *out_len, int *status, int level, int strategy, int hash_variant,
                            void *hip_stream) {
    if (!check_args(c, n, in_len, level, strategy)) return ZS_STREAM_ERROR;
    if (n == 0) return ZS_OK;
    if (hipSetDevice(c->device) != hipSuccess) return ZS_STREAM_ERROR;
    hipStream_t s = hip_stream ? (hipStream_t)hip_stream : c->stream;
    int rc = ZS_OK;
    for (int lo = 0; lo < n;) {
        const int hi = batch_prefix_that_fits(c, n, in_len, out_cap, lo, 19);
        if (!run_pipeline(c, hi - lo, in + lo, in_len + lo, out + lo, out_cap + lo, out_len + lo, status ? status + lo : nullptr, level, strategy,
                          hash_variant, s) && rc == ZS_OK)
            rc = c->err == "buffer error" ? ZS_BUF_ERROR : ZS_STREAM_ERROR;
        lo = hi;
    }
    return rc;
}

int zs_deflate_writes_batch_device(zs_ctx *c, int n, const void *const *in, const int64_t *in_len, const int64_t *const *write_ends,
                                   const int64_t *n_writes, void *const *out, const int64_t *out_cap, int64_t *out_len, int *status, int level,
                                   int strategy, int hash_variant, void *hip_stream) {
    if (!write_ends) return zs_deflate_batch_device(c, n, in, in_len, out, out_cap, out_len, status, level, strategy, hash_variant, hip_stream);
    if (!check_args(c, n, in_len, level, strategy)) return ZS_STREAM_ERROR;
    if (n == 0) return ZS_OK;
    std::vector<WriteSpec> specs((size_t)n);
    std::vector<const WriteSpec *> ptrs((size_t)n, nullptr);
    for (int i = 0; i < n; i++) {
        if (!write_ends[i] || (n_writes && n_writes[i] <= 0)) continue;
        if (!n_writes || !write_list_ends(write_ends[i], n_writes[i], in_len[i], specs[(size_t)i].ends)) {
            c->err = "stream error";
            return ZS_STREAM_ERROR;
        }
        if (specs[(size_t)i].ends.empty()) continue;
        specs[(size_t)i].flush.assign(specs[(size_t)i].ends.size(), 0);
        ptrs[(size_t)i] = &specs[(size_t)i];
    }
    if (hipSetDevice(c->device) != hipSuccess) return ZS_STREAM_ERROR;
    hipStream_t s = hip_stream ? (hipStream_t)hip_stream : c->stream;
    int rc = ZS_OK;
    for (int lo = 0; lo < n;) {
        const int hi = batch_prefix_that_fits(c, n, in_len, out_cap, lo, 19);
        if (!run_pipeline(c, hi - lo, in + lo, in_len + lo, out + lo, out_cap + lo, out_len + lo, status ? status + lo : nullptr, level, strategy,
                          hash_variant, s, ptrs.data() + lo) && rc == ZS_OK)
            rc = c->err == "buffer error" ? ZS_BUF_ERROR : ZS_STREAM_ERROR;
        lo = hi;
    }
    return rc;
}

int zs_deflate_writes_device(zs_ctx *c, const void *in, int64_t in_len, const int64_t *write_ends, int64_t n_writes, void *out,
                             int64_t out_cap, int64_t *out_len, int level, int strategy, int hash_variant, void *hip_stream) {
    if (!check_args(c, 1, &in_len, level, strategy)) return ZS_STREAM_ERROR;
    if (hipSetDevice(c->device) != hipSuccess) return ZS_STREAM_ERROR;
    WriteSpec ws;
    if (!write_list_ends(write_ends, n_writes, in_len, ws.ends)) {
        c->err = "stream error";
        return ZS_STREAM_ERROR;
    }
    ws.flush.assign(ws.ends.size(), 0);
    const WriteSpec *const one = &ws;
    hipStream_t s = hip_stream ? (hipStream_t)hip_stream : c->stream;
    int st = 0;
    if (!run_pipeline(c, 1, &in, &in_len, &out, &out_cap, out_len, &st, level, strategy, hash_variant, s, ws.ends.size() > 1 ? &one : nullptr))
        return c->err == "buffer error" ? ZS_BUF_ERROR : ZS_STREAM_ERROR;
    return ZS_OK;
}

namespace {
int deflate_batch_host_once(zs_ctx *c, int n, const void *const *in, const int64_t *in_len, void *const *out, const int64_t *out_cap,
                            int64_t *out_len, int *status, int level, int strategy, int hash_variant) {
    std::vector<const void *> din((size_t)n);
    std::vector<void *> dout((size_t)n);
    std::vector<int64_t> dcap((size_t)n);
    size_t tin = 0, tout = 0;
    for (int i = 0; i < n; i++) {
        tin += ((size_t)in_len[i] + 255) & ~(size_t)255;
        dcap[(size_t)i] = out_cap[i];
        tout += ((size_t)out_cap[i] + 255) & ~(size_t)255;
    }
    auto chk = [&](hipError_t e, const char *what) {
        if (e != hipSuccess) fail(c, what, e);
        return e == hipSuccess;
    };
    if (!ensure(c, c->stage_in, tin + 256) || !ensure(c, c->stage_out, tout + 256)) return ZS_MEM_ERROR;
    size_t oi = 0, oo = 0;
    for (int i = 0; i < n; i++) {
        din[(size_t)i] = (uint8_t *)c->stage_in.p + oi;
        dout[(size_t)i] = (uint8_t *)c->stage_out.p + oo;
        if (in_len[i] &&
            !chk(hipMemcpyAsync((void *)din[(size_t)i], in[i], (size_t)in_len[i], hipMemcpyHostToDevice, c->stream), "H2D"))
            return ZS_STREAM_ERROR;
        oi += ((size_t)in_len[i] + 255) & ~(size_t)255;
        oo += ((size_t)out_cap[i] + 255) & ~(size_t)255;
    }
    std::vector<int> st_local;
    if (!status) st_local.assign((size_t)n, 0), status = st_local.data();
    const bool ok = run_pipeline(c, n, din.data(), in_len, dout.data(), dcap.data(), out_len, status, level, strategy, hash_variant, c->stream);
    const std::string first_err = c->err;
    for (int i = 0; i < n; i++)
        if (status[i] == 0 && out_len[i] > 0 && out_len[i] <= out_cap[i] &&
            !chk(hipMemcpyAsync(out[i], dout[(size_t)i], (size_t)out_len[i], hipMemcpyDeviceToHost, c->stream), "D2H"))
            return ZS_STREAM_ERROR;
    if (!chk(hipStreamSynchronize(c->stream), "sync")) return ZS_STREAM_ERROR;
    if (!ok) {
        c->err = first_err;
        return first_err == "buffer error" ? ZS_BUF_ERROR : ZS_STREAM_ERROR;
    }
    return ZS_OK;
}
}

int zs_deflate_batch(zs_ctx *c, int n, const void *const *in, const int64_t *in_len, void *const *out, const int64_t *out_cap,
                     int64_t *out_len, int *status, int level, int strategy, int hash_variant) {
    if (!check_args(c, n, in_len, level, strategy)) return ZS_STREAM_ERROR;
    if (n == 0) return ZS_OK;
    if (hipSetDevice(c->device) != hipSuccess) return ZS_STREAM_ERROR;
    int rc = ZS_OK;
    std::string first_err;
    for (int lo = 0; lo < n;) {
        const int hi = batch_prefix_that_fits(c, n, in_len, out_cap, lo, 20);
        const int r = deflate_batch_host_once(c, hi - lo, in + lo, in_len + lo, out + lo, out_cap + lo, out_len + lo, status ? status + lo : nullptr, level,
                                              strategy, hash_variant);
        if (r != ZS_OK && rc == ZS_OK) rc = r, first_err = c->err;
        lo = hi;
    }
    if (rc != ZS_OK) c->err = first_err;
    return rc;
}

int zs_adler32_device(zs_ctx *c, const void *d_buf, int64_t len, uint32_t seed, uint32_t *out, void *hip_stream) {
    if (!c || !out || len < 0 || len > 0x7FFFFFFF - 1024) return ZS_STREAM_ERROR;
    if (hipSetDevice(c->device) != hipSuccess) return ZS_STREAM_ERROR;
    hipStream_t s = hip_stream ? (hipStream_t)hip_stream : c->stream;
    uint32_t ad = 1;
    if (!device_adlers(c, 1, &d_buf, &len, nullptr, &ad, nullptr, s)) return ZS_STREAM_ERROR;
    *out = adler_combine(seed, ad, (uint64_t)len);
    return ZS_OK;
}

}


namespace {
const char *const kInfMessages[kInfMsgCount] = {
    "", "unknown compression method", "invalid window size", "incorrect header check", "need dictionary", "invalid block type",
    "invalid stored block lengths", "too many length or distance symbols", "invalid bit length repeat",
    "oversubscribed dynamic bit lengths tree", "incomplete dynamic bit lengths tree", "oversubscribed literal/length tree",
    "incomplete literal/length tree", "oversubscribed distance tree", "incomplete distance tree", "empty distance tree with lengths",
    "invalid literal/length code", "invalid distance code", "buffer error", "buffer error", "incorrect data check"};

bool run_inflate_seq(zs_ctx *c, int n, const void *const *in, const int64_t *in_len, void *const *out, const int64_t *out_cap,
                 int64_t *out_len, int *status, hipStream_t stream, uint32_t *adler_out = nullptr, int *msg_out = nullptr) {
    std::vector<InfDesc> d((size_t)n);
    for (int i = 0; i < n; i++) d[(size_t)i] = {(const uint8_t *)in[i], (uint8_t *)out[i], in_len[i], out_cap[i]};
    if (!ensure(c, c->inf_desc, sizeof(InfDesc) * (size_t)n) || !ensure(c, c->inf_state, sizeof(InfState) * (size_t)n)) return false;
    std::vector<InfState> st((size_t)n);
    ZS_HIP(c, hipMemcpyAsync(c->inf_desc.p, d.data(), sizeof(InfDesc) * (size_t)n, hipMemcpyHostToDevice, stream));
    ZS_HIP(c, hipStreamSynchronize(stream));
    const bool prof = c->profiling;
    if (prof) (void)hipEventRecord(c->ev[0], stream);
    hipLaunchKernelGGL(zs_inflate_kernel, dim3((unsigned)n), dim3(64), kInfLds, stream, dev<InfDesc>(c->inf_desc),
                       dev<InfState>(c->inf_state));
    if (prof) (void)hipEventRecord(c->ev[1], stream);
    ZS_HIP(c, hipGetLastError());
    ZS_HIP(c, hipMemcpyAsync(st.data(), c->inf_state.p, sizeof(InfState) * (size_t)n, hipMemcpyDeviceToHost, stream));
    ZS_HIP(c, hipStreamSynchronize(stream));
    if (prof) {
        float ms = 0;
        (void)hipEventElapsedTime(&ms, c->ev[0], c->ev[1]);
        for (double &v : c->stage_ms) v = 0;
        c->stage_ms[0] = ms;
    }
    std::vector<const void *> abuf;
    std::vector<int64_t> alen;
    std::vector<int> aidx;
    for (int i = 0; i < n; i++)
        if (st[(size_t)i].status == ZS_STREAM_END) abuf.push_back(out[i]), alen.push_back(st[(size_t)i].out_len), aidx.push_back(i);
    if (c->inf_probe == nullptr && n == 1) c->inf_used.assign(1, st[0].status == ZS_STREAM_END ? st[0].in_used : 0);
    std::vector<uint32_t> ads(abuf.size(), 1u);
    if (!device_adlers(c, (int)abuf.size(), abuf.data(), alen.data(), nullptr, ads.data(), nullptr, stream)) return false;
    for (size_t k = 0; k < aidx.size(); k++) {
        InfState &q = st[(size_t)aidx[k]];
        if (ads[k] != q.adler_stored) q.status = ZS_DATA_ERROR, q.msg = kInfBadCheck;
        else if (adler_out) adler_out[aidx[k]] = ads[k];
    }
    bool all_ok = true;
    for (int i = 0; i < n; i++) {
        out_len[i] = st[(size_t)i].out_len;
        const int code = st[(size_t)i].status;
        if (status) status[i] = code;
        if (msg_out) msg_out[i] = st[(size_t)i].msg;
        if (code != ZS_STREAM_END) {
            if (all_ok) c->err = kInfMessages[st[(size_t)i].msg];
            all_ok = false;
        }
    }
    return all_ok;
}

bool run_inflate_piece(zs_ctx *c, const void *in, int64_t in_len, bool first, int64_t start_bit, const void *hist, int hist_have, void *out, int64_t out_cap,
                       int64_t *out_len, int64_t *good_bits, int64_t *in_used, int *status, uint32_t *adler_stored, hipStream_t stream) {
    InfDesc d{(const uint8_t *)in, (uint8_t *)out, in_len, out_cap, (const uint8_t *)hist, first ? 0 : start_bit, hist_have, first ? 1 : 2};
    if (!ensure(c, c->inf_desc, sizeof(InfDesc)) || !ensure(c, c->inf_state, sizeof(InfState))) return false;
    InfState st;
    ZS_HIP(c, hipMemcpyAsync(c->inf_desc.p, &d, sizeof d, hipMemcpyHostToDevice, stream));
    ZS_HIP(c, hipStreamSynchronize(stream));
    hipLaunchKernelGGL(zs_inflate_kernel, dim3(1), dim3(64), kInfLds, stream, dev<InfDesc>(c->inf_desc), dev<InfState>(c->inf_state));
    ZS_HIP(c, hipGetLastError());
    ZS_HIP(c, hipMemcpyAsync(&st, c->inf_state.p, sizeof st, hipMemcpyDeviceToHost, stream));
    ZS_HIP(c, hipStreamSynchronize(stream));
    *out_len = st.out_len, *good_bits = st.good_bits, *in_used = st.in_used, *status = st.status, *adler_stored = st.adler_stored;
    if (st.status != ZS_OK && st.status != ZS_STREAM_END) c->err = kInfMessages[st.msg];
    return true;
}

constexpr int64_t kParMinInput = 1024;

bool run_inflate_par(zs_ctx *c, const std::vector<int> &idx, const void *const *in, const int64_t *in_len, void *const *out,
                     const int64_t *out_cap, int64_t *out_len, int *status, hipStream_t stream, std::vector<int> &rest,
                     uint32_t *adler_out = nullptr, int *msg_out = nullptr) {
    const int m = (int)idx.size();
    c->inf_lane_streams = 0;
    c->inf_wave_streams = 0;
    if (m == 0) return true;
    std::vector<ParStream> ps((size_t)m);
    int64_t nchunks = 0, ncand = 0, nblk = 0, ncells = 0, nfx = 0;
    std::vector<uint2> w_find;
    for (int j = 0; j < m; j++) {
        const int i = idx[(size_t)j];
        ParStream &p = ps[(size_t)j];
        p.in = (const uint8_t *)in[i], p.out = (uint8_t *)out[i], p.in_len = in_len[i], p.out_cap = out_cap[i];
        p.chunk_off = (int32_t)nchunks, p.nchunks = (int32_t)((in_len[i] + kFindChunk - 1) / kFindChunk);
        nchunks += p.nchunks;
        p.cand_off = (int32_t)ncand, p.max_cand = (int32_t)(in_len[i] / 128 + 64);
        ncand += p.max_cand;
        p.blk_off = (int32_t)nblk, p.max_blk = (int32_t)(in_len[i] / 96 + 64);
        nblk += p.max_blk;
        p.cell_off = ncells;
        p.fx_off = (int32_t)nfx, p.fx_regions = (int32_t)(in_len[i] * 8 / kFxRegionBits + 1);
        nfx += p.fx_regions;
        if (c->inf_probe) p.out_cap = (int64_t)0x7FFFFFFF - 1024;
        else ncells += (out_cap[i] + 63) & ~63LL;
        for (int k = 0; k < p.nchunks; k++) w_find.push_back(make_uint2((unsigned)j, (unsigned)k));
    }
    if (!ensure(c, c->par_ps, sizeof(ParStream) * (size_t)m) || !ensure(c, c->par_st, sizeof(ParState) * (size_t)m) ||
        !ensure(c, c->par_work, sizeof(uint2) * (size_t)std::max<int64_t>(std::max<int64_t>(nchunks, ncand), nblk) + 64) ||
        !ensure(c, c->par_cbits, 8 * (size_t)nchunks * kFindMaxCand + 64) || !ensure(c, c->par_ccnt, 4 * (size_t)nchunks + 64) ||
        !ensure(c, c->par_surv, 4 * (size_t)nchunks * kFindMaxSurv + 64) || !ensure(c, c->par_scnt, 4 * (size_t)nchunks + 64) ||
        !ensure(c, c->par_cands, sizeof(ParCand) * (size_t)ncand) || !ensure(c, c->par_blocks, sizeof(ParBlock) * (size_t)nblk) ||
        !ensure(c, c->par_cells, 2 * (size_t)ncells + 64) || !ensure(c, c->par_fail, 4 * (size_t)m + 64))
        return false;
    std::vector<ParState> st((size_t)m);
    ZS_HIP(c, hipMemcpyAsync(c->par_ps.p, ps.data(), sizeof(ParStream) * (size_t)m, hipMemcpyHostToDevice, stream));
    ZS_HIP(c, hipMemcpyAsync(c->par_work.p, w_find.data(), sizeof(uint2) * w_find.size(), hipMemcpyHostToDevice, stream));
    ZS_HIP(c, hipMemsetAsync(c->par_fail.p, 0, 4 * (size_t)m + 64, stream));
    ZS_HIP(c, hipStreamSynchronize(stream));
    const ParStream *d_ps = dev<ParStream>(c->par_ps);
    ParState *d_st = dev<ParState>(c->par_st);
    const bool prof = c->profiling;
    auto mark = [&](int k) {
        if (prof) (void)hipEventRecord(c->ev[k], stream);
    };
    mark(0);
// ... 2832 lines not shown
```

Baseline: 15440 MB/s.

## Cache host-side compression plan across calls and merge descriptor uploads

Adds a plan cache keyed on stream count, lengths, capacities, level, strategy and relevant environment settings. When the key matches and no buffer was reallocated, the host planning step is skipped and only the per-call input/output pointers are patched and uploaded. Stream descriptors, worklist prefixes and geometry now go up in one pinned transfer instead of three. The spec-compact kernel is also queued before the host waits on the verdict flags, using an event instead of a full stream sync, so the GPU keeps working during the host readback. The cost is extra state, with a risk of stale-plan bugs if some planning input is missing from the key.

Result: faster. 15880 MB/s, median of 6 (+2.9%).

```diff
diff --git a/zlibstream_amd/csrc/zs_engine.hip b/zlibstream_amd/csrc/zs_engine.hip
--- a/zlibstream_amd/csrc/zs_engine.hip
+++ b/zlibstream_amd/csrc/zs_engine.hip
@@ -15,6 +15,7 @@
 #include "zs_inflate_tok.hip"
 #include "zs_png.hip"
 #include "zs_crc32.hip"
+#include "zs_plan_key.h"
 
 using namespace zs;
 
@@ -32,6 +33,8 @@
 const char *const kStageNames[kStCount] = {"clear", "adler", "links", "match", "chunkmap", "segmap", "resolve", "expand",
                                            "emit_syms", "tail", "trees", "offsets", "emit_bits", "spec_walk", "spec_verify", "crc32_frame",
                                            "spec_compact", "png_expand", "png_split", "png_pack", "png_survey", "png_compose", "png_diff", "png_crop"};
+
+struct PlanCache;
 
 }
 
@@ -62,7 +65,7 @@
     hipEvent_t ev[kStCount + 1] = {};
     double stage_ms[kStCount] = {};
     uint32_t *crc_tab = nullptr;
-    DevBuf sd, st, work, wpre, geo, link, mm, maps, chunk_far, segmap, supmap, seg_entry, seg_symbase, seg_stale, entry, symbase, stale, syms, blk_end, blk_top, blocks, trees, info, tile_bits, pieces, scratch,
+    DevBuf sd, st, work, link, mm, maps, chunk_far, segmap, supmap, seg_entry, seg_symbase, seg_stale, entry, symbase, stale, syms, blk_end, blk_top, blocks, trees, info, tile_bits, pieces, scratch,
         stage_in, stage_out, wr, inf_desc, inf_state, par_ps, par_st, par_work, par_cbits, par_ccnt, par_surv, par_scnt, par_cands, par_tabs, par_toktabs, par_toks, par_ctoks, par_tokstat, par_tails, par_retry, par_fxtab, par_blocks, par_cells,
         par_windows, par_fail, run_syms, run_bits, run_scratch, run_outs, run_fail, adl_tr, adl_res, plan_blk, ins_bits, mm_bak, cut_pos, cut_bkt, win_groups, win_sg, win_maps, win_entries, persist_bak, resume_flag, rle_tiles, own_in, fr_chunks, fr_meta, fr_planes, fr_prov, fr_base, fr_counters, spec_rec, spec_flags, spec_syms, png_img, png_seg, png_ctr, png_fimg, png_scratch, png_a7img, png_inflated, png_passes, crc_desc, crc_res, png_zs, png_gather, png_ximg, png_raw, png_simg, png_split, png_gimg, png_vimg, png_vrec, png_packed, png_cimg, png_frames, png_dimg, png_drec, png_kimg, png_crop;
     uint32_t *crc32_tab = nullptr;
@@ -83,6 +86,12 @@
     void *pin_out = nullptr;
     size_t pin_out_cap = 0;
     bool pin_out_busy = false;
+    PlanCache *plan = nullptr;
+    void *plan_pin = nullptr;
+    size_t plan_pin_cap = 0;
+    uint64_t plan_gen = 0;
+    int plan_reused = 0;
+    hipEvent_t ev_verdict = nullptr;
 };
 
 namespace {
@@ -99,6 +108,7 @@
 
 bool ensure(zs_ctx *c, DevBuf &b, size_t bytes) {
     if (bytes <= b.cap) return true;
+    c->plan_gen++;
     if (b.p) (void)hipFree(b.p);
     b.p = nullptr;
     b.cap = 0;
@@ -117,6 +127,15 @@
         }
     }
     b.cap = want;
+    return true;
+}
+bool ensure_plan_pin(zs_ctx *c, size_t bytes) {
+    if (bytes <= c->plan_pin_cap) return true;
+    if (c->plan_pin) (void)hipHostFree(c->plan_pin);
+    c->plan_pin = nullptr;
+    c->plan_pin_cap = 0;
+    ZS_HIP(c, hipHostMalloc(&c->plan_pin, bytes + bytes / 8 + 4096, hipHostMallocDefault));
+    c->plan_pin_cap = bytes + bytes / 8 + 4096;
     return true;
 }
 bool ensure_pinned(zs_ctx *c, size_t bytes) {
@@ -164,6 +183,21 @@
     std::vector<int32_t> plan_wr_blk;
 };
 
+struct PlanCache {
+    PlanKey key, probe;
+    Plan pl;
+    bool valid = false;
+    uint64_t gen = 0;
+    bool in_flight = false;
+    size_t o[kWorkLists] = {};
+    int64_t link_span = 0;
+    bool dual_saved = false;
+    std::vector<StreamDesc> dual_sd;
+    std::vector<FsChunk> dual_fr;
+    int dual_fr_max_n = 0;
+    int64_t dual_n_runs = 0;
+};
+
 template <class T>
 T *dev(DevBuf &b) {
     return (T *)b.p;
@@ -217,6 +251,35 @@
                 c->err = "flush modes and incremental runs take one stream a call";
                 return false;
             }
+    if (!c->plan) c->plan = new PlanCache();
+    PlanCache &pc = *c->plan;
+    const bool no_rounds_this_call = c->no_rounds_once;
+    c->no_rounds_once = false;
+    c->fast_rounds = 0;
+    c->plan_reused = 0;
+    bool plan_hit = false, plan_keep = false;
+    {
+        bool flush_any = false;
+        std::vector<PlanWritesView> views;
+        std::vector<const PlanWritesView *> view_ptrs;
+        if (any_writes) {
+            views.resize((size_t)n), view_ptrs.assign((size_t)n, nullptr);
+            for (int i = 0; i < n; i++) {
+                const WriteSpec *wr = writes[i];
+                if (!wr) continue;
+                flush_any = flush_any || wr->flushing() || wr->flush.size() != wr->ends.size();
+                views[(size_t)i] = PlanWritesView{wr->ends.data(), wr->flush.data(), wr->ends.size(), wr->chunk, wr->raw};
+                view_ptrs[(size_t)i] = &views[(size_t)i];
+            }
+        }
+        plan_keep = !ro && !rounds && !force_lit && !no_rounds_this_call && force_seq == 0 && level != 0 && !flush_any && !getenv("ZS_NO_PLAN_REUSE");
+        if (plan_keep) {
+            plan_key_fill(pc.probe, n, in_len, out_cap, level, strategy, hash_variant, force_seq, ro != nullptr, rounds, force_lit != nullptr, no_rounds_this_call,
+                          any_writes ? view_ptrs.data() : nullptr, plan_env_read());
+            plan_hit = pc.valid && pc.gen == c->plan_gen && !pc.in_flight && plan_key_equal(pc.key, pc.probe);
+        }
+        if (!plan_hit) pc.valid = false, pc.dual_saved = false, c->plan_gen++;
+    }
     std::vector<WriteSpec> rle_one;
     std::vector<const WriteSpec *> rle_writes;
     if (any_writes && strategy == kRle && level >= 1 && !ro && !getenv("ZS_NO_RLE_MULTI")) {
@@ -250,12 +313,17 @@
     const int spec_warm = getenv("ZS_SPEC_WARM") ? std::max(0, std::min(4096, atoi(getenv("ZS_SPEC_WARM")))) : kSpecWarm;
     const int64_t spec_min = getenv("ZS_SPEC_MIN") ? std::max<int64_t>(kWindowSize, atoll(getenv("ZS_SPEC_MIN"))) : kSpecMinInput;
     const int spec_corrupt = getenv("ZS_SPEC_CORRUPT") ? atoi(getenv("ZS_SPEC_CORRUPT")) : -1;
+    Plan &pl = pc.pl;
+    size_t &o_clear = pc.o[0], &o_adler = pc.o[1], &o_links = pc.o[2], &o_match = pc.o[3], &o_chunks = pc.o[4], &o_segs = pc.o[5], &o_sups = pc.o[6],
+           &o_blocks = pc.o[7], &o_runs = pc.o[8];
+    auto plan_call = [&]() -> bool {
 plan_again:
-    Plan pl;
+    pl = Plan();
     pl.sd.resize((size_t)n);
     int64_t total_len = 0;
     for (int i = 0; i < n; i++) total_len += in_len[i];
     const int64_t link_span = total_len >= (48ll << 20) ? 262144 : total_len >= (24ll << 20) ? 131072 : 65536;
+    pc.link_span = link_span;
     const int run_chunk = getenv("ZS_FAST_CHUNK") ? std::max(65536, std::min((int)kFastChunk, atoi(getenv("ZS_FAST_CHUNK")) & ~65535))
                                                   : (int)std::max<int64_t>(65536, std::min<int64_t>(kFastChunk, ((total_len / 256 + 65535) >> 16) << 16));
     for (int i = 0; i < n; i++) {
@@ -449,11 +517,6 @@
         goto plan_again;
     }
     pl.any_dual = allow_dual;
-    c->lit_engine_bytes += pl.lit_bytes;
-    auto plan_rerun = [&]() { c->lit_engine_bytes -= pl.lit_bytes; };
-    c->fast_rounds = 0;
-    const bool no_rounds_this_call = c->no_rounds_once;
-    c->no_rounds_once = false;
     if (pl.any_fv && !getenv("ZS_FAST_NO_ROUNDS") && !no_rounds_this_call && !(ro && ro->resume && getenv("ZS_NO_RESUME_ROUNDS"))) {
         int64_t pos_fv = 0, max_fv = 0;
         for (int i = 0; i < n; i++)
@@ -506,9 +569,14 @@
     }
     WorkList *const lists[kWorkLists] = {&pl.w_clear, &pl.w_adler, &pl.w_links, &pl.w_match, &pl.w_chunks, &pl.w_segs, &pl.w_sups, &pl.w_blocks, &pl.w_runs};
     for (WorkList *l : lists) l->finish(n);
-    size_t n_work = pl.w_clear.size() + pl.w_adler.size() + pl.w_links.size() + pl.w_match.size() + pl.w_chunks.size() +
-                    pl.w_segs.size() + pl.w_sups.size() + pl.w_blocks.size() + pl.w_runs.size();
-    if (!ensure(c, c->sd, sizeof(StreamDesc) * (size_t)n) || !ensure(c, c->st, sizeof(StreamState) * (size_t)n) ||
+    const size_t n_work = pl.w_clear.size() + pl.w_adler.size() + pl.w_links.size() + pl.w_match.size() + pl.w_chunks.size() +
+                          pl.w_segs.size() + pl.w_sups.size() + pl.w_blocks.size() + pl.w_runs.size();
+    const size_t o_segcl = 16 * (size_t)pl.n_segs, o_cstart = o_segcl + 4 * ((size_t)pl.n_segs + (size_t)n),
+                 o_head = o_cstart + 4 * ((size_t)pl.n_chunks + (size_t)n), o_cl = o_head + 4 * (size_t)pl.n_chunks;
+    const size_t geo_bytes = o_cl + 4 * pl.cl.size();
+    const size_t sd_bytes = sizeof(StreamDesc) * (size_t)n, pre_bytes = 4 * (size_t)kWorkLists * (size_t)(n + 1);
+    const size_t up_bytes = sd_bytes + pre_bytes + geo_bytes;
+    if (!ensure(c, c->sd, up_bytes + 64) || !ensure(c, c->st, sizeof(StreamState) * (size_t)n) ||
         !ensure(c, c->work, sizeof(uint2) * (n_work + 1)) || !ensure(c, c->link, 2 * (size_t)pl.n_pos + 64) ||
         !ensure(c, c->mm, 8 * (size_t)pl.n_pos + 256) ||
         !ensure(c, c->maps, 4 * (size_t)(pl.n_chunks + 1) * kSlots) || !ensure(c, c->segmap, 8 * (size_t)(pl.n_segs + 1) * kSlots) ||
@@ -525,14 +593,10 @@
         (pl.n_spec && (!ensure(c, c->spec_rec, 8 * (size_t)pl.n_spec + 64) || !ensure(c, c->spec_flags, 4 * (size_t)n + 64) ||
                        !ensure(c, c->spec_syms, 4 * (size_t)pl.n_spec * (size_t)spec_slab_stride(spec_bits) + 64))))
         return false;
-    const size_t o_segcl = 16 * (size_t)pl.n_segs, o_cstart = o_segcl + 4 * ((size_t)pl.n_segs + (size_t)n),
-                 o_head = o_cstart + 4 * ((size_t)pl.n_chunks + (size_t)n), o_cl = o_head + 4 * (size_t)pl.n_chunks;
-    const size_t geo_bytes = o_cl + 4 * pl.cl.size();
-    if (!ensure(c, c->geo, geo_bytes + 64)) return false;
     for (int i = 0; i < n; i++) {
         StreamDesc &s = pl.sd[(size_t)i];
-        const int32_t *g = (const int32_t *)c->geo.p;
-        const uint8_t *gb = (const uint8_t *)c->geo.p;
+        const uint8_t *gb = (const uint8_t *)c->sd.p + sd_bytes + pre_bytes;
+        const int32_t *g = (const int32_t *)gb;
         s.seg_c0 = g + s.seg_off, s.seg_after = g + pl.n_segs + s.seg_off, s.seg_base = g + 2 * pl.n_segs + s.seg_off;
         s.seg_S = g + 3 * pl.n_segs + s.seg_off;
         s.seg_cl = (const int32_t *)(gb + o_segcl) + s.seg_off + i;
@@ -588,19 +652,15 @@
         ZS_HIP(c, hipMemcpyAsync(c->plan_blk.p, pl.plan_blk.data(), sizeof(BlockRec) * pl.plan_blk.size(), hipMemcpyHostToDevice, stream));
         ZS_HIP(c, hipStreamSynchronize(stream));
     }
-    const size_t pre_bytes = 4 * (size_t)kWorkLists * (size_t)(n + 1);
-    size_t up_bytes = sizeof(StreamDesc) * (size_t)n + pre_bytes + geo_bytes + 16;
-    if (!ensure_pinned(c, std::max(up_bytes, sizeof(StreamState) * (size_t)n)) || !ensure(c, c->wpre, pre_bytes + 64)) return false;
-    uint8_t *hp = (uint8_t *)c->pinned;
-    memcpy(hp, pl.sd.data(), sizeof(StreamDesc) * (size_t)n);
-    int32_t *hpre = (int32_t *)(hp + sizeof(StreamDesc) * (size_t)n);
-    size_t o_clear = 0, o_adler, o_links, o_match, o_chunks, o_segs, o_sups, o_blocks, o_runs;
+    if (!ensure_pinned(c, std::max(sd_bytes + 16, sizeof(StreamState) * (size_t)n)) || !ensure_plan_pin(c, up_bytes + 16)) return false;
+    uint8_t *hp = (uint8_t *)c->plan_pin;
+    memcpy(hp, pl.sd.data(), sd_bytes);
+    int32_t *hpre = (int32_t *)(hp + sd_bytes);
     WorkOffsets wo;
     {
-        size_t *const offs[kWorkLists] = {&o_clear, &o_adler, &o_links, &o_match, &o_chunks, &o_segs, &o_sups, &o_blocks, &o_runs};
         size_t at = 0;
         for (int l = 0; l < kWorkLists; l++) {
-            *offs[l] = at;
+            pc.o[l] = at;
             wo.off[l] = (uint32_t)at;
             memcpy(hpre + (size_t)l * (size_t)(n + 1), lists[l]->pre.data(), 4 * (size_t)(n + 1));
             at += lists[l]->size();
@@ -608,7 +668,7 @@
         wo.off[kWorkLists] = (uint32_t)at;
     }
     if (geo_bytes) {
-        uint8_t *hg = hp + sizeof(StreamDesc) * (size_t)n + pre_bytes;
+        uint8_t *hg = hp + sd_bytes + pre_bytes;
         if (pl.n_segs) {
             memcpy(hg, pl.seg_c0.data(), 4 * (size_t)pl.n_segs);
             memcpy(hg + 4 * (size_t)pl.n_segs, pl.seg_after.data(), 4 * (size_t)pl.n_segs);
@@ -619,15 +679,34 @@
         memcpy(hg + o_cstart, pl.cstart.data(), 4 * pl.cstart.size());
         if (pl.n_chunks) memcpy(hg + o_head, pl.head.data(), 4 * (size_t)pl.n_chunks);
         if (!pl.cl.empty()) memcpy(hg + o_cl, pl.cl.data(), 4 * pl.cl.size());
-        if (!rounds) ZS_HIP(c, hipMemcpyAsync(c->geo.p, hg, geo_bytes, hipMemcpyHostToDevice, stream));
-    }
-    if (!rounds) ZS_HIP(c, hipMemcpyAsync(c->sd.p, hp, sizeof(StreamDesc) * (size_t)n, hipMemcpyHostToDevice, stream));
-    if (n_work && !rounds) {
-        ZS_HIP(c, hipMemcpyAsync(c->wpre.p, hpre, pre_bytes, hipMemcpyHostToDevice, stream));
-        hipLaunchKernelGGL(zs_worklist_kernel, dim3((unsigned)((n_work + 255) / 256)), dim3(256), 0, stream, dev<int32_t>(c->wpre), n, wo,
-                           dev<uint2>(c->work));
     }
     if (!rounds) {
+        pc.in_flight = true;
+        ZS_HIP(c, hipMemcpyAsync(c->sd.p, hp, up_bytes, hipMemcpyHostToDevice, stream));
+        if (n_work)
+            hipLaunchKernelGGL(zs_worklist_kernel, dim3((unsigned)((n_work + 255) / 256)), dim3(256), 0, stream,
+                               (const int32_t *)((const uint8_t *)c->sd.p + sd_bytes), n, wo, dev<uint2>(c->work));
+    }
+    return true;
+    };
+    if (plan_hit) {
+        c->plan_reused = 1;
+        if (pc.dual_saved) pl.sd = pc.dual_sd, pl.fr_chunks = pc.dual_fr, pl.fr_max_n = pc.dual_fr_max_n, pl.n_runs = pc.dual_n_runs, pl.any_fv = true;
+        StreamDesc *hd = (StreamDesc *)c->plan_pin;
+        for (int i = 0; i < n; i++) {
+            hd[i].in = pl.sd[(size_t)i].in = (const uint8_t *)in[i];
+            hd[i].out = pl.sd[(size_t)i].out = (uint8_t *)out[i];
+        }
+        pc.in_flight = true;
+        ZS_HIP(c, hipMemcpyAsync(c->sd.p, hd, sizeof(StreamDesc) * (size_t)n, hipMemcpyHostToDevice, stream));
+    } else {
+        if (!plan_call()) return false;
+        if (plan_keep) std::swap(pc.key, pc.probe), pc.valid = true, pc.gen = c->plan_gen;
+    }
+    const int64_t link_span = pc.link_span;
+    c->lit_engine_bytes += pl.lit_bytes;
+    auto plan_rerun = [&]() { c->lit_engine_bytes -= pl.lit_bytes; };
+    auto zero_state = [&]() -> bool {
         ZeroRegions z;
         auto reg = [&](int r, DevBuf &b, size_t bytes) {
             z.p[r] = b.p;
@@ -649,7 +728,8 @@
             if (hi > lo) ZS_HIP(c, hipMemsetAsync(pl.sd[0].ins_bits + lo, 0xFF, (size_t)(hi - lo) * 4, stream));
             ZS_HIP(c, hipMemsetD32Async((hipDeviceptr_t)(pl.sd[0].ins_bits + hi), (int)((1u << (ro->p0 & 31)) - 1u), 1, stream));
         }
-    }
+        return true;
+    };
 
     const StreamDesc *d_sd = dev<StreamDesc>(c->sd);
     StreamState *d_st = dev<StreamState>(c->st);
@@ -762,11 +842,15 @@
         }
         return true;
     };
+    const bool tail_late = ro && (!ro->final_run || ro->resume);
+    const bool tail_serial = !tail_late && n >= 64 && (pl.n_pos / n >= (96 << 10) || getenv("ZS_TAIL_SERIAL")) && !getenv("ZS_TAIL_FORK");
+    bool fork_recorded = false;
     if (!rounds) {
     mark(2);
     if (!pl.w_links.empty())
         hipLaunchKernelGGL(zs_links_kernel, dim3((unsigned)pl.w_links.size()), dim3(1024), kLkLds, stream, d_sd, d_work + o_links,
                            dev<uint16_t>(c->link), c->crc_tab, hash_variant, (int)link_span);
+    if (!zero_state()) return false;
     if (ro && ro->resume)
         hipLaunchKernelGGL(zs_import_chains_kernel, dim3(64), dim3(1024), 0, stream, d_sd, 0, dev<uint16_t>(c->link), c->crc_tab, hash_variant, ro->p0);
     if (pl.any_dual) {
@@ -778,6 +862,7 @@
             ZS_HIP(c, hipStreamSynchronize(stream));
             for (int i = 0; i < n; i++) periodic = periodic && np[(size_t)i] == 0;
         }
+        if (pc.valid && !pc.dual_saved) pc.dual_saved = true, pc.dual_sd = pl.sd, pc.dual_fr = pl.fr_chunks, pc.dual_fr_max_n = pl.fr_max_n, pc.dual_n_runs = pl.n_runs;
         for (int i = 0; i < n; i++) {
             StreamDesc &sk = pl.sd[(size_t)i];
             if (periodic) sk.fv_end = -1, sk.fr_first = 0, sk.fr_n = 0;
@@ -807,7 +892,16 @@
                            strategy, hash_variant, k5s, dev<int32_t>(c->spec_flags));
         int32_t *hf = (int32_t *)c->pinned;
         ZS_HIP(c, hipMemcpyAsync(hf, c->spec_flags.p, 4 * (size_t)n, hipMemcpyDeviceToHost, stream));
-        ZS_HIP(c, hipStreamSynchronize(stream));
+        ZS_HIP(c, hipEventRecord(c->ev_verdict, stream));
+        if (!tail_late && !tail_serial) {
+            ZS_HIP(c, hipEventRecord(c->ev_fork, stream));
+            fork_recorded = true;
+        }
+        if (prof) (void)hipEventRecord(c->ev_spec[2], stream);
+        hipLaunchKernelGGL(zs_spec_compact_kernel, dim3((unsigned)((pl.max_spec_n + 3) / 4), (unsigned)n), dim3(256), 0, stream, d_sd, d_st, k5s,
+                           dev<uint32_t>(c->syms), dev<int32_t>(c->blk_end), dev<int32_t>(c->blk_top));
+        if (prof) (void)hipEventRecord(c->ev_spec[3], stream);
+        ZS_HIP(c, hipEventSynchronize(c->ev_verdict));
         if (prof) (void)hipEventRecord(c->ev_spec[1], stream);
         for (int i = 0; i < n; i++) {
             if (hf[i] == 0) continue;
@@ -932,10 +1026,8 @@
             hipLaunchKernelGGL(zs_rle_pass_kernel<1>, tg, dim3(256), 0, stream, d_sd, rt, dev<uint32_t>(c->syms), dev<int32_t>(c->blk_end), dev<int32_t>(c->blk_top), s0);
         });
     }
-    const bool tail_late = ro && (!ro->final_run || ro->resume);
-    const bool tail_serial = !tail_late && n >= 64 && (pl.n_pos / n >= (96 << 10) || getenv("ZS_TAIL_SERIAL")) && !getenv("ZS_TAIL_FORK");
     if (!tail_late && !tail_serial) {
-        ZS_HIP(c, hipEventRecord(c->ev_fork, stream));
+        if (!fork_recorded || need_maps) ZS_HIP(c, hipEventRecord(c->ev_fork, stream));
         ZS_HIP(c, hipStreamWaitEvent(c->aux, c->ev_fork, 0));
         hipLaunchKernelGGL(zs_tail_kernel, dim3((unsigned)n), dim3(1024), kTailLds, c->aux, d_sd, d_st, dev<uint16_t>(c->link),
                            dev<uint32_t>(c->syms), dev<int32_t>(c->blk_end), dev<int32_t>(c->blk_top), dev<BlockRec>(c->blocks),
@@ -954,12 +1046,6 @@
                            d_work + o_chunks, (int)pl.w_chunks.size(), dev<uint2>(c->mm), dev<uint16_t>(c->link), dev<uint16_t>(c->entry),
                            dev<uint32_t>(c->symbase), dev<uint32_t>(c->syms), dev<int32_t>(c->blk_end), dev<int32_t>(c->blk_top),
                            c->crc_tab, lv, strategy, hash_variant, k5_ahead, k5s);
-    if (spec_ok_streams) {
-        if (prof) (void)hipEventRecord(c->ev_spec[2], stream);
-        hipLaunchKernelGGL(zs_spec_compact_kernel, dim3((unsigned)((pl.max_spec_n + 3) / 4), (unsigned)n), dim3(256), 0, stream, d_sd, d_st, k5s,
-                           dev<uint32_t>(c->syms), dev<int32_t>(c->blk_end), dev<int32_t>(c->blk_top));
-        if (prof) (void)hipEventRecord(c->ev_spec[3], stream);
-    }
     mark(9);
     if (tail_serial)
         hipLaunchKernelGGL(zs_tail_kernel, dim3((unsigned)n), dim3(1024), kTailLds, stream, d_sd, d_st, dev<uint16_t>(c->link),
@@ -1031,8 +1117,9 @@
     mark(10);
     const int trees_threads = pl.w_blocks.size() > 8192 ? 128 : 256;
     if (n >= 64 && !getenv("ZS_NO_LIVE_LIST")) {
-        hipLaunchKernelGGL(zs_live_scan_kernel, dim3(1), dim3(1024), 0, stream, d_st, n, dev<int32_t>(c->wpre));
-        hipLaunchKernelGGL(zs_live_fill_kernel, dim3((unsigned)((pl.w_blocks.size() + 255) / 256)), dim3(256), 0, stream, dev<int32_t>(c->wpre), n,
+        int32_t *const d_live = (int32_t *)((uint8_t *)c->sd.p + sizeof(StreamDesc) * (size_t)n);
+        hipLaunchKernelGGL(zs_live_scan_kernel, dim3(1), dim3(1024), 0, stream, d_st, n, d_live);
+        hipLaunchKernelGGL(zs_live_fill_kernel, dim3((unsigned)((pl.w_blocks.size() + 255) / 256)), dim3(256), 0, stream, d_live, n,
                            (uint32_t)pl.w_blocks.size(), dev<uint2>(c->work) + o_blocks);
     }
     hipLaunchKernelGGL(zs_trees_kernel, dim3((unsigned)pl.w_blocks.size()), dim3(trees_threads), 0, stream, d_sd, d_st, d_work + o_blocks,
@@ -1059,7 +1146,11 @@
     ZS_HIP(c, hipMemcpyAsync(hst, d_st, sizeof(StreamState) * (size_t)n, hipMemcpyDeviceToHost, stream));
     ht_launched = ht_us();
     ZS_HIP(c, hipStreamSynchronize(stream));
-    if (host_times) fprintf(stderr, "zs: host: plan + uploads %.0f us, all launched at %.0f us, device done at %.0f us\n", ht_plan, ht_launched, ht_us());
+    pc.in_flight = false;
+    if (pc.valid && !plan_hit) pc.gen = c->plan_gen;
+    if (host_times)
+        fprintf(stderr, "zs: host: plan + uploads %.0f us%s, all launched at %.0f us, device done at %.0f us\n", ht_plan, c->plan_reused ? " (kept plan)" : "", ht_launched,
+                ht_us());
     c->last_op = lv.func == 1 ? 2 : 0;
     if (getenv("ZS_DEBUG_CHAIN") && n == 1) {
         const int64_t q0 = atoll(getenv("ZS_DEBUG_CHAIN")) - (ro ? ro->abs_off : 0);
@@ -1103,8 +1194,9 @@
             (void)hipEventElapsedTime(&m, c->ev_spec[1], c->ev[kStChunkMap + 1]);
             c->stage_ms[kStSpecWalk] = a, c->stage_ms[kStSpecVerify] = b, c->stage_ms[kStChunkMap] = m;
             float k = 0;
-            if (spec_ok_streams) (void)hipEventElapsedTime(&k, c->ev_spec[2], c->ev_spec[3]);
+            (void)hipEventElapsedTime(&k, c->ev_spec[2], c->ev_spec[3]);
             c->stage_ms[kStSpecCompact] = k;
+            c->stage_ms[kStSpecVerify] = b > k ? b - k : 0;
         }
     }
     {
@@ -1150,6 +1242,7 @@
 bool device_adlers(zs_ctx *c, int m, const void *const *bufs, const int64_t *lens, const void *const *trailers, uint32_t *adlers,
                    int *ok, hipStream_t stream) {
     if (m <= 0) return true;
+    c->plan_gen++;
     std::vector<StreamDesc> sd((size_t)m);
     std::vector<uint2> work;
     int64_t n_pieces = 0;
@@ -1270,7 +1363,8 @@
         hipEventCreateWithFlags(&c->ev_fork, hipEventDisableTiming) != hipSuccess ||
         hipEventCreateWithFlags(&c->ev_join, hipEventDisableTiming) != hipSuccess ||
         hipEventCreateWithFlags(&c->ev_pre0, hipEventDisableTiming) != hipSuccess ||
-        hipEventCreateWithFlags(&c->ev_pre, hipEventDisableTiming) != hipSuccess) {
+        hipEventCreateWithFlags(&c->ev_pre, hipEventDisableTiming) != hipSuccess ||
+        hipEventCreateWithFlags(&c->ev_verdict, hipEventDisableTiming) != hipSuccess) {
         zs_ctx_destroy(c);
         return ZS_MEM_ERROR;
     }
@@ -1310,7 +1404,7 @@
 void zs_ctx_destroy(zs_ctx *c) {
     if (!c) return;
     (void)hipSetDevice(c->device);
-    DevBuf *bufs[] = {&c->sd, &c->st, &c->work, &c->wpre, &c->geo, &c->link, &c->mm, &c->maps, &c->chunk_far, &c->segmap, &c->supmap, &c->seg_entry, &c->seg_symbase, &c->seg_stale, &c->entry, &c->symbase, &c->stale, &c->syms,
+    DevBuf *bufs[] = {&c->sd, &c->st, &c->work, &c->link, &c->mm, &c->maps, &c->chunk_far, &c->segmap, &c->supmap, &c->seg_entry, &c->seg_symbase, &c->seg_stale, &c->entry, &c->symbase, &c->stale, &c->syms,
                       &c->blk_end, &c->blk_top, &c->blocks, &c->trees, &c->info, &c->tile_bits, &c->pieces, &c->scratch, &c->stage_in, &c->stage_out, &c->wr, &c->inf_desc, &c->inf_state, &c->par_ps, &c->par_st, &c->par_work, &c->par_cbits, &c->par_ccnt, &c->par_surv, &c->par_scnt,
                       &c->par_cands, &c->par_tabs, &c->par_toktabs, &c->par_toks, &c->par_ctoks, &c->par_tokstat, &c->par_tails, &c->par_retry, &c->par_fxtab, &c->par_blocks, &c->par_cells, &c->par_windows, &c->par_fail, &c->run_syms, &c->run_bits,
                       &c->run_scratch, &c->run_outs, &c->run_fail, &c->adl_tr, &c->adl_res, &c->plan_blk, &c->ins_bits, &c->mm_bak, &c->cut_pos, &c->cut_bkt, &c->win_groups, &c->win_sg, &c->win_maps, &c->win_entries, &c->persist_bak, &c->resume_flag, &c->rle_tiles, &c->own_in, &c->fr_chunks, &c->fr_meta, &c->fr_planes, &c->fr_prov, &c->fr_base, &c->fr_counters, &c->spec_rec, &c->spec_flags, &c->spec_syms, &c->png_img, &c->png_seg, &c->png_ctr, &c->png_fimg, &c->png_scratch, &c->png_a7img, &c->png_inflated, &c->png_passes, &c->crc_desc, &c->crc_res, &c->png_zs, &c->png_gather, &c->png_ximg, &c->png_raw, &c->png_simg, &c->png_split, &c->png_gimg, &c->png_vimg, &c->png_vrec, &c->png_packed, &c->png_cimg, &c->png_frames, &c->png_dimg, &c->png_drec, &c->png_kimg, &c->png_crop};
@@ -1335,6 +1429,9 @@
     for (auto &e : c->ev_crop)
         if (e) (void)hipEventDestroy(e);
     if (c->pinned) (void)hipHostFree(c->pinned);
+    if (c->plan_pin) (void)hipHostFree(c->plan_pin);
+    delete c->plan;
+    if (c->ev_verdict) (void)hipEventDestroy(c->ev_verdict);
     if (c->pin_io) (void)hipHostFree(c->pin_io);
     if (c->pin_out) (void)hipHostFree(c->pin_out);
     for (auto &e : c->ev)
@@ -1371,6 +1468,7 @@
     if (k == "spec_fallbacks") return c->spec_fallbacks;
     if (k == "spec_periodic") return c->spec_periodic;
     if (k == "spec_wrong_chunks") return c->spec_wrong_chunks;
+    if (k == "plan_reused") return c->plan_reused;
     if (k == "inf_lane_streams") return c->inf_lane_streams;
     if (k == "inf_wave_streams") return c->inf_wave_streams;
     if (k == "png_segments") return c->png_segments;
diff --git a/zlibstream_amd/csrc/zs_plan_key.h b/zlibstream_amd/csrc/zs_plan_key.h
--- /dev/null
+++ b/zlibstream_amd/csrc/zs_plan_key.h
@@ -0,0 +1,95 @@
+#pragma once
+#include <cstdint>
+#include <cstdlib>
+#include <vector>
+
+namespace zs {
+
+struct PlanEnv {
+    bool no_rle_multi = false, no_fast_vec = false, fast_no_rounds = false, no_spec = false, no_fast_multi = false, no_fast_resume = false,
+         no_rle_runs = false, no_resume_rounds = false, no_live_list = false;
+    bool has_fr_ratio = false, has_fr_chunk = false, has_fast_chunk = false;
+    int spec_len = 0;
+    int spec_warm = -1, fast_chunk = 0;
+    int64_t spec_min = -1, fr_chunk = 0;
+    double fr_ratio = 0;
+};
+inline PlanEnv plan_env_read() {
+    PlanEnv e;
+    auto on = [](const char *k) { return getenv(k) != nullptr; };
+    e.no_rle_multi = on("ZS_NO_RLE_MULTI"), e.no_fast_vec = on("ZS_NO_FAST_VEC"), e.fast_no_rounds = on("ZS_FAST_NO_ROUNDS");
+    e.no_spec = on("ZS_NO_SPEC"), e.no_fast_multi = on("ZS_NO_FAST_MULTI"), e.no_fast_resume = on("ZS_NO_FAST_RESUME");
+    e.no_rle_runs = on("ZS_NO_RLE_RUNS"), e.no_resume_rounds = on("ZS_NO_RESUME_ROUNDS");
+    e.no_live_list = on("ZS_NO_LIVE_LIST");
+    if (const char *v = getenv("ZS_SPEC_LEN")) e.spec_len = atoi(v);
+    if (const char *v = getenv("ZS_SPEC_WARM")) e.spec_warm = atoi(v);
+    if (const char *v = getenv("ZS_SPEC_MIN")) e.spec_min = atoll(v);
+    if (const char *v = getenv("ZS_FAST_CHUNK")) e.has_fast_chunk = true, e.fast_chunk = atoi(v);
+    if (const char *v = getenv("ZS_FR_CHUNK")) e.has_fr_chunk = true, e.fr_chunk = atoll(v);
+    if (const char *v = getenv("ZS_FR_RATIO")) e.has_fr_ratio = true, e.fr_ratio = atof(v);
+    return e;
+}
+inline bool plan_env_equal(const PlanEnv &a, const PlanEnv &b) {
+    return a.no_rle_multi == b.no_rle_multi && a.no_fast_vec == b.no_fast_vec && a.fast_no_rounds == b.fast_no_rounds && a.no_spec == b.no_spec &&
+           a.no_fast_multi == b.no_fast_multi && a.no_fast_resume == b.no_fast_resume && a.no_rle_runs == b.no_rle_runs &&
+           a.no_resume_rounds == b.no_resume_rounds && a.no_live_list == b.no_live_list && a.has_fr_ratio == b.has_fr_ratio && a.has_fr_chunk == b.has_fr_chunk &&
+           a.has_fast_chunk == b.has_fast_chunk && a.spec_len == b.spec_len && a.spec_warm == b.spec_warm && a.fast_chunk == b.fast_chunk &&
+           a.spec_min == b.spec_min && a.fr_chunk == b.fr_chunk && a.fr_ratio == b.fr_ratio;
+}
+
+struct PlanKeyWrites {
+    bool present = false, raw = false;
+    int chunk = 512;
+    std::vector<int64_t> ends;
+    std::vector<uint8_t> flush;
+};
+inline bool plan_writes_equal(const PlanKeyWrites &a, const PlanKeyWrites &b) {
+    return a.present == b.present && a.raw == b.raw && a.chunk == b.chunk && a.ends == b.ends && a.flush == b.flush;
+}
+
+struct PlanKey {
+    int n = 0, level = 0, strategy = 0, hash_variant = 0;
+    int force_seq = 0;
+    bool incremental = false, rounds = false, forced_lit = false, no_rounds = false;
+    std::vector<int64_t> in_len, out_cap;
+    std::vector<PlanKeyWrites> writes;
+    PlanEnv env;
+};
+inline bool plan_key_reusable(const PlanKey &k) { return !k.incremental && !k.rounds && !k.forced_lit && !k.no_rounds && k.force_seq == 0; }
+inline bool plan_key_equal(const PlanKey &a, const PlanKey &b) {
+    if (!plan_key_reusable(a) || !plan_key_reusable(b)) return false;
+    if (a.n != b.n || a.level != b.level || a.strategy != b.strategy || a.hash_variant != b.hash_variant || a.force_seq != b.force_seq) return false;
+    if (a.in_len != b.in_len || a.out_cap != b.out_cap || a.writes.size() != b.writes.size()) return false;
+    for (size_t i = 0; i < a.writes.size(); i++)
+        if (!plan_writes_equal(a.writes[i], b.writes[i])) return false;
+    return plan_env_equal(a.env, b.env);
+}
+
+struct PlanWritesView {
+    const int64_t *ends = nullptr;
+    const uint8_t *flush = nullptr;
+    size_t n_ends = 0;
+    int chunk = 512;
+    bool raw = false;
+};
+inline void plan_key_fill(PlanKey &k, int n, const int64_t *in_len, const int64_t *out_cap, int level, int strategy, int hash_variant, int force_seq,
+                          bool incremental, bool rounds, bool forced_lit, bool no_rounds, const PlanWritesView *const *writes, const PlanEnv &env) {
+    k.n = n, k.level = level, k.strategy = strategy, k.hash_variant = hash_variant, k.force_seq = force_seq;
+    k.incremental = incremental, k.rounds = rounds, k.forced_lit = forced_lit, k.no_rounds = no_rounds;
+    k.in_len.assign(in_len, in_len + n);
+    k.out_cap.assign(out_cap, out_cap + n);
+    bool any = false;
+    for (int i = 0; i < n && writes; i++) any = any || writes[i] != nullptr;
+    k.writes.resize(any ? (size_t)n : 0);
+    for (size_t i = 0; i < k.writes.size(); i++) {
+        PlanKeyWrites &w = k.writes[i];
+        const PlanWritesView *v = writes[i];
+        w.present = v != nullptr;
+        w.raw = v && v->raw, w.chunk = v ? v->chunk : 512;
+        if (v) w.ends.assign(v->ends, v->ends + v->n_ends), w.flush.assign(v->flush, v->flush + v->n_ends);
+        else w.ends.clear(), w.flush.clear();
+    }
+    k.env = env;
+}
+
+}
```
